# Fabstir/fabstir-vectordb

Hardware: AMD Instinct MI355X
Metric: k-NN queries/sec at recall@10>=0.95, 1Mx384 f32 (higher is better)
Workload: dtype f32

## Files before the change

fabstir-vectordb_amd/_capi.py:

```python
import ctypes as C
import os

_HERE = os.path.dirname(os.path.abspath(__file__))
LIB_DIR = os.environ.get("FVDB_LIB_DIR") or os.path.join(_HERE, "lib")
if not os.path.isabs(LIB_DIR):
    LIB_DIR = os.path.join(_HERE, LIB_DIR)
LIB_PATH = os.environ.get("FVDB_HIP_LIB") or os.path.join(LIB_DIR, "libfvdb_hip.so")

vp, u64, u32, i32, f32, sz = C.c_void_p, C.c_uint64, C.c_uint32, C.c_int, C.c_float, C.c_size_t
f32p, u64p, u32p = C.POINTER(C.c_float), C.POINTER(C.c_uint64), C.POINTER(C.c_uint32)


class TrainResult(C.Structure):
    _fields_ = [("iterations", u32), ("converged", u32), ("initial_error", f32), ("final_error", f32)]


class SearchStats(C.Structure):
    _fields_ = [("rows_scanned", u64), ("work_items", u64), ("list_rows_touched", u64)]


class MaskInfo(C.Structure):
    _fields_ = [("kind", u32), ("stale", u32), ("units", u32), ("reserved", u32), ("allowed_live", u64)]


# ... 23 lines not shown
    "fvdb_dev_upload": (i32, [vp, vp, vp, sz]),
    "fvdb_dev_download": (i32, [vp, vp, vp, sz]),
    "fvdb_timer_start": (i32, [vp]),
    "fvdb_timer_stop_ms": (i32, [vp, f32p]),
    "fvdb_ctx_set_profiling": (i32, [vp, i32]),
    "fvdb_dot_products": (i32, [vp, f32p, u32, f32p, u64, u32, f32p]),
    "fvdb_cosine_similarities": (i32, [vp, f32p, u32, f32p, u64, u32, f32p]),
    "fvdb_ivf_create": (i32, [vp, u32, u32, C.POINTER(vp)]),
    "fvdb_ivf_create_ex": (i32, [vp, u32, u32, i32, C.POINTER(vp)]),
    "fvdb_ivf_destroy": (None, [vp]),
    "fvdb_ivf_set_centroids": (i32, [vp, f32p]),
    "fvdb_ivf_get_centroids": (i32, [vp, f32p]),
    "fvdb_ivf_train": (i32, [vp, f32p, u64, u32, u64, C.POINTER(TrainResult)]),
    "fvdb_ivf_assign": (i32, [vp, f32p, u64, u32p]),
    "fvdb_ivf_add": (i32, [vp, f32p, u64p, u64, u32p, u32p]),
    "fvdb_ivf_add_assigned": (i32, [vp, f32p, u64p, u64, u32p, u32p]),
    "fvdb_ivf_set_deleted": (i32, [vp, u32p, u32p, u64, i32]),
    "fvdb_ivf_list_sizes": (i32, [vp, u64p]),
    "fvdb_ivf_list_export": (i32, [vp, u32, f32p, u64p, C.POINTER(C.c_uint8)]),
    "fvdb_ivf_total_rows": (u64, [vp]),
    "fvdb_ivf_reserve": (i32, [vp, u64]),
    "fvdb_ivf_clear": (i32, [vp]),
    "fvdb_ivf_set_global_list_sizes": (i32, [vp, u64p]),
    "fvdb_ivf_compact": (i32, [vp, u64p, u64p]),
    "fvdb_ivf_train_from": (i32, [vp, vp, u32, u64, C.POINTER(TrainResult)]),
    "fvdb_ivf_assign_from": (i32, [vp, vp, u32p, u64p]),
    "fvdb_ivf_refill_from": (i32, [vp, vp, u64, u32p]),
    "fvdb_ivf_maintenance_info": (i32, [vp, C.POINTER(MaintenanceInfo)]),
    "fvdb_ivf_get_rows": (i32, [vp, u32p, u32p, u64, f32p]),
    "fvdb_ivf_get_rows_dev": (i32, [vp, vp, u32p, u32p, u64, vp]),
    "fvdb_ivf_assign_from_store": (i32, [vp, vp, u32p, u64, u32p]),
    "fvdb_ivf_add_assigned_from_store": (i32, [vp, vp, u32p, u64p, u64, u32p, u32p]),
    "fvdb_ivf_search": (i32, [vp, f32p, u32, u32, u32, u64p, f32p, u32p]),
    "fvdb_ivf_search_dev": (i32, [vp, vp, u32, u32, u32, vp, vp, vp, vp]),
    "fvdb_ivf_search_all": (i32, [vp, f32p, u32, u32, u64p, f32p, u32p]),
    "fvdb_ivf_search_all_dev": (i32, [vp, vp, u32, u32, vp, vp, vp]),
    "fvdb_ivf_coarse": (i32, [vp, f32p, u32, u32, u32p, f32p]),
    "fvdb_ivf_set_coarse_mode": (i32, [vp, i32]),
    "fvdb_ivf_coarse_fallbacks": (i32, [vp, u64p]),
    "fvdb_ivf_set_scan_mode": (i32, [vp, i32]),
    "fvdb_ivf_scan_fallbacks": (i32, [vp, u64p]),
    "fvdb_ivf_scan_fallback_reasons": (i32, [vp, u64p]),
    "fvdb_ivf_scan_survivors": (i32, [vp, u32p, u32]),
    "fvdb_ivf_scan_survivor_dump": (i32, [vp, u32, u32, u32p, u32p, f32p, u32p]),
    "fvdb_ivf_last_stats": (i32, [vp, C.POINTER(SearchStats)]),
    "fvdb_ivf_stage_times": (u64, [vp, f32p]),
    "fvdb_ivf_profile_collect": (i32, [vp]),
    "fvdb_merge_keys_dev": (i32, [vp, vp, vp, u32, u32, u32, vp, vp, vp]),
    "fvdb_store_create": (i32, [vp, u32, u64, C.POINTER(vp)]),
    "fvdb_store_destroy": (None, [vp]),
    "fvdb_store_append": (i32, [vp, f32p, u64, u64p]),
    "fvdb_store_rows": (u64, [vp]),
    "fvdb_store_get": (i32, [vp, u64, f32p]),
    "fvdb_score_candidates": (i32, [vp, f32p, u32, u32p, u32, f32p]),
    "fvdb_scorer_create": (i32, [vp, u32, u32, C.POINTER(vp)]),
    "fvdb_scorer_destroy": (None, [vp]),
    "fvdb_scorer_set_queries": (i32, [vp, f32p, u32]),
    "fvdb_scorer_set_query_rows": (i32, [vp, u32p, u32]),
    "fvdb_scorer_set_queries_dev": (i32, [vp, vp, u32]),
    "fvdb_scorer_cand_buffer": (u32p, [vp]),
    "fvdb_scorer_dist_buffer": (f32p, [vp]),
    "fvdb_scorer_run": (i32, [vp, u32, u32]),
    "fvdb_graph_create": (i32, [vp, C.POINTER(vp)]),
    "fvdb_graph_destroy": (None, [vp]),
    "fvdb_graph_upload": (i32, [vp, u32, u32p, C.POINTER(C.c_uint8), u32p, u32p, u32]),
    "fvdb_graph_set_deleted": (i32, [vp, u32, i32]),
    "fvdb_graph_configure": (i32, [vp, u32, u32]),
    "fvdb_graph_append_nodes": (i32, [vp, u32, u32, u32p]),
    "fvdb_graph_insert_linked": (i32, [vp, u32, u32, u32, i32, u32p, vp]),
    "fvdb_graph_set_lists": (i32, [vp, u32, u32p, u32p, u32p, u32p]),
    "fvdb_graph_set_entry": (i32, [vp, u32, u32]),
    "fvdb_graph_entry": (i32, [vp, u32p, u32p]),
    "fvdb_graph_download": (i32, [vp, u32p, u32p, u64, u64p]),
    "fvdb_graph_upload_bytes": (u64, [vp]),
    "fvdb_graph_set_insert_visited": (i32, [vp, i32, u32]),
    "fvdb_graph_insert_info": (i32, [vp, u32, vp]),
    "fvdb_graph_vacuum": (i32, [vp, u32, u64p]),
    "fvdb_graph_maintenance_info": (i32, [vp, C.POINTER(GraphMaintenanceInfo)]),
    "fvdb_graph_search_dev": (i32, [vp, vp, u32, u32, u32, vp, vp, vp, vp]),
    "fvdb_graph_search_dev_slot": (i32, [vp, vp, u32, vp, u32, u32, u32, vp, vp, vp, vp]),
    "fvdb_ctx_device": (i32, [vp]),
    "fvdb_ctx_info": (i32, [vp, vp]),
    "fvdb_ivf_search_dev_slot": (i32, [vp, vp, u32, vp, u32, u32, u32, vp, vp, vp, vp]),
    "fvdb_ivf_coarse_dev_slot": (i32, [vp, vp, u32, vp, u32, u32, vp]),
    "fvdb_ivf_search_probes_dev_slot": (i32, [vp, vp, u32, vp, vp, u32, u32, u32, vp, vp, vp, vp]),
    "fvdb_host_alloc": (i32, [vp, C.c_size_t, C.POINTER(vp)]),
    "fvdb_host_free": (None, [vp, vp]),
    "fvdb_dev_download_async": (i32, [vp, vp, vp, C.c_size_t]),
    "fvdb_event_create": (i32, [vp, C.POINTER(vp)]),
    "fvdb_event_destroy": (None, [vp]),
    "fvdb_event_record": (i32, [vp, vp]),
    "fvdb_event_wait": (i32, [vp, vp]),
    "fvdb_graph_kernel_times": (i32, [vp, f32p, u32p, u64p, u64p]),
    "fvdb_graph_tie_restarts": (i32, [vp, u64p, u64p]),
    "fvdb_scorer_launch": (i32, [vp, u32, u32]),
    "fvdb_scorer_wait": (i32, [vp]),
    "fvdb_top_k_indices": (i32, [vp, f32p, u32, u64, u32, u64p, u32p]),
    "fvdb_top_k_indices_heap": (i32, [vp, f32p, u32, u64, u32, u64p, u32p]),
    "fvdb_top_k_indices_dev": (i32, [vp, vp, u32, u64, u32, i32, vp, vp]),
    "fvdb_streaming_top_k": (i32, [vp, u64p, f32p, u32, u64, u32, u64p, f32p, u32p]),
    "fvdb_streaming_top_k_dev": (i32, [vp, vp, vp, u32, u64, u32, vp, vp, vp]),
    "fvdb_merge_search_results": (i32, [vp, u64p, f32p, u32, u64, u32, u64p, f32p, u32p]),
    "fvdb_merge_search_results_dev": (i32, [vp, vp, vp, u32, u64, u32, vp, vp, vp]),
    "fvdb_comm_unique_id": (i32, [vp]),
    "fvdb_comm_create": (i32, [vp, vp, i32, i32, C.POINTER(vp)]),
    "fvdb_comm_create_hosted": (i32, [vp, i32, i32, vp, vp, C.POINTER(vp)]),
    "fvdb_comm_destroy": (None, [vp]),
    "fvdb_comm_rank": (i32, [vp]),
    "fvdb_comm_world": (i32, [vp]),
    "fvdb_comm_all_gather_dev": (i32, [vp, vp, vp, vp, sz]),
    "fvdb_comm_all_to_all_dev": (i32, [vp, vp, vp, vp, sz]),
    "fvdb_sharded_create": (i32, [vp, vp, C.POINTER(vp)]),
    "fvdb_sharded_destroy": (None, [vp]),
    "fvdb_sharded_out_rows": (u32, [vp, u32, i32]),
    "fvdb_ivf_search_sharded_begin": (i32, [vp, vp, u32, vp, u32, u32, u32, i32, vp, vp, vp]),
    "fvdb_ivf_search_sharded_end": (i32, [vp, vp, u32]),
    "fvdb_mask_create_ivf": (i32, [vp, u64p, u64, C.POINTER(vp)]),
    "fvdb_mask_create_graph": (i32, [vp, u32p, u64, C.POINTER(vp)]),
    "fvdb_mask_info": (i32, [vp, vp]),
    "fvdb_mask_destroy": (None, [vp]),
    "fvdb_ivf_search_dev_slot_masked": (i32, [vp, vp, u32, vp, vp, u32, u32, u32, vp, vp, vp, vp]),
    "fvdb_ivf_search_probes_dev_slot_masked": (i32, [vp, vp, u32, vp, vp, vp, u32, u32, u32, vp, vp, vp, vp]),
    "fvdb_ivf_search_wide_dev_slot": (i32, [vp, vp, u32, vp, vp, u32, u32, u32, vp, vp, vp, vp]),
    "fvdb_ivf_search_wide": (i32, [vp, f32p, u32, u32, u32, u64p, f32p, u32p]),
    "fvdb_ivf_search_quality_dev": (i32, [vp, vp, u32, vp, u32, u32, u32, vp, vp]),
    "fvdb_graph_search_dev_slot_masked": (i32, [vp, vp, u32, vp, vp, u32, u32, u32, vp, vp, vp, vp]),
    "fvdb_graph_scan_allowed_dev_slot": (i32, [vp, vp, u32, vp, vp, u32, u32, vp, vp, vp]),
}

_lib = None


def load():
    global _lib
    if _lib is not None:
        return _lib
    if not os.path.exists(LIB_PATH):
        raise ImportError(
            f"{LIB_PATH} not found: build it with `make -C fabstir-vectordb_amd` "
            "(or __graft_entry__.build()).  There is no CPU fallback.")
    os.environ.setdefault("GPU_MAX_HW_QUEUES", "16")
    lib = C.CDLL(LIB_PATH)
    for name, (res, args) in SIGNATURES.items():
        fn = getattr(lib, name)
        fn.restype = res
        fn.argtypes = args
    _lib = lib
    return lib
```

fabstir-vectordb_amd/csrc/fvdb_hip.cpp:

```cpp
#include "fvdb_internal.h"

#include <unistd.h>

#include <algorithm>
#include <atomic>
#include <cmath>
#include <condition_variable>
#include <mutex>
#include <cstdio>
#include <cstdlib>
#include <cstring>
#include <map>
#include <new>
#include <string>
#include <vector>

#include "common.h"
#include "kernels_misc.h"
#include "kernels_scan.h"
#include "kernels_wide.h"
#include "kernels_rank.h"
#include "kernels_coarse.h"
#include "kernels_mfma.h"
#include "kernels_mfma_wg.h"
// ... 40 lines not shown
    uint64_t* nv = nullptr;
    float* nn = nullptr;
    HIPCHK(ctx, hipMalloc(&nd, (size_t)ncap * block_bytes()));
    HIPCHK(ctx, hipMemsetAsync(nd, 0, (size_t)ncap * block_bytes(), ctx->stream));
    float* nr = nullptr;
    if (mirror && esize == 4) {
      HIPCHK(ctx, hipMalloc((void**)&nr, (size_t)ncap * block_bytes()));
      HIPCHK(ctx, hipMemsetAsync(nr, 0, (size_t)ncap * block_bytes(), ctx->stream));
      if (used_blocks && rm)
        HIPCHK(ctx, hipMemcpyAsync(nr, rm, (size_t)used_blocks * block_bytes(), hipMemcpyDeviceToDevice, ctx->stream));
    }
    void* nh = nullptr;
    if (mirror) {
      HIPCHK(ctx, hipMalloc(&nh, (size_t)ncap * block_bytes() / 2));
      HIPCHK(ctx, hipMemsetAsync(nh, 0, (size_t)ncap * block_bytes() / 2, ctx->stream));
      if (used_blocks && half)
        HIPCHK(ctx, hipMemcpyAsync(nh, half, (size_t)used_blocks * block_bytes() / 2, hipMemcpyDeviceToDevice, ctx->stream));
    }
    HIPCHK(ctx, hipMalloc(&nn, (size_t)ncap * 64 * sizeof(float)));
    HIPCHK(ctx, hipMemsetAsync(nn, 0, (size_t)ncap * 64 * sizeof(float), ctx->stream));
    HIPCHK(ctx, hipMalloc(&ni, (size_t)ncap * 64 * sizeof(uint64_t)));
    HIPCHK(ctx, hipMalloc(&nv, (size_t)ncap * sizeof(uint64_t)));
    HIPCHK(ctx, hipMemsetAsync(nv, 0, (size_t)ncap * sizeof(uint64_t), ctx->stream));
    if (used_blocks) {
      HIPCHK(ctx, hipMemcpyAsync(nd, data, (size_t)used_blocks * block_bytes(), hipMemcpyDeviceToDevice, ctx->stream));
      HIPCHK(ctx, hipMemcpyAsync(ni, ids, (size_t)used_blocks * 64 * sizeof(uint64_t), hipMemcpyDeviceToDevice,
                                 ctx->stream));
      HIPCHK(ctx, hipMemcpyAsync(nv, valid, (size_t)used_blocks * sizeof(uint64_t), hipMemcpyDeviceToDevice,
                                 ctx->stream));
      HIPCHK(ctx, hipMemcpyAsync(nn, norms, (size_t)used_blocks * 64 * sizeof(float), hipMemcpyDeviceToDevice,
                                 ctx->stream));
    }
    HIPCHK(ctx, hipStreamSynchronize(ctx->stream));
    if (data) (void)hipFree(data);
    if (ids) (void)hipFree(ids);
    if (valid) (void)hipFree(valid);
    if (norms) (void)hipFree(norms);
    if (half) (void)hipFree(half);
    half = nh;
    if (rm) (void)hipFree(rm);
    rm = nr;
    norms = nn;
    data = nd;
    ids = ni;
    valid = nv;
    cap_blocks = ncap;
    return FVDB_OK;
  }
};

enum FbWord : uint32_t {
  FB_COARSE = 0,
  FB_SCAN = 1,
  FB_REASONS = 2,
  FB_OVERFLOW = 2,
  FB_REFINED = 6,
  FB_WORDS = 8,
};
constexpr size_t kFbBytes = FB_WORDS * 4;
constexpr size_t kFbAllBytes = 2 * kFbBytes;
constexpr uint32_t kFbReasonWords = 5;

enum StageEvent {
  EV_COARSE_BEGIN = 0,
  EV_COARSE_SCANNED,
  EV_COARSE_DONE,
  EV_SCAN_BEGIN,
  EV_SCAN_DONE,
  EV_FINE_DONE,
  EV_FILTER_BEGIN,
  EV_FILTER_DONE,
  EV_COUNT
};

enum ScalWord : uint32_t {
  SC_COARSE_ITEMS = 0,
  SC_COARSE_HEAD = 1,
  SC_FINE_ITEMS = 2,
  SC_FINE_HEAD = 3,
  SC_STATS = 4,
};
constexpr size_t kScalarsBytes = 64;

struct IvfScratch {
  std::mutex enq;
  bool pend_filter = false;
  bool pending_profile = false, pend_coarse = false, pend_fine = false, collecting = false;
  std::vector<DBuf*> bufs;
  struct Buf : DBuf {
    explicit Buf(IvfScratch* set) { set->bufs.push_back(this); }
  };
  Buf s_qnorm{this}, s_A{this};
  Buf s_qh{this}, s_qn2{this}, s_thr{this}, s_tA{this}, s_pa{this}, s_surv{this}, s_scnt{this}, s_fail{this}, s_mslots{this};
  Buf s_sdist{this}, s_probes2{this};
  Buf s_q{this}, s_cpart{this}, s_probes{this}, s_cnt{this}, s_fill{this}, s_eoff{this}, s_ioff{this}, s_entries{this};
  Buf s_part{this}, s_scalars{this}, s_ceoff{this}, s_cioff{this};
  Buf s_wbase{this}, s_arena{this};
  Buf s_rbase{this}, s_rarena{this};
  Buf s_qual{this};
  Buf s_in{this}, s_slots{this}, s_ids{this}, s_clusters{this}, s_out_ids{this}, s_out_dist{this}, s_out_cnt{this}, s_cdist{this};
  Buf s_fslots{this}, s_frows{this};
  hipEvent_t fetch_done = nullptr;
  hipEvent_t sev[EV_COUNT] = {};
  uint32_t* scalar(ScalWord w) const { return s_scalars.as<uint32_t>() + w; }
  void release_all() {
    for (DBuf* b : bufs) b->release();
    if (fetch_done) (void)hipEventDestroy(fetch_done);
    fetch_done = nullptr;
    for (auto& e : sev) {
      if (e) (void)hipEventDestroy(e);
      e = nullptr;
    }
  }
};

struct fvdb_ivf : IvfScratch {
  static constexpr uint32_t kSlots = 16;
  IvfScratch spare[kSlots - 1];
  static constexpr uint32_t kLeases = 8;
  IvfScratch lease_set[kLeases];
  fvdb_ctx* lease_ctx[kLeases] = {};
  uint32_t lease_busy = 0;
  std::mutex mu;
  std::condition_variable lease_cv;
  std::atomic<IvfScratch*> last_set{nullptr};
  std::atomic<fvdb_ctx*> last_ctx{nullptr};
  fvdb_ctx* ctx = nullptr;
  uint32_t d = 0, dpad = 0, d4 = 0, nlist = 0;
  bool trained = false;
  bool f16 = false;

  std::vector<float> h_centroids;
  DBuf d_centroids_rm;
  DBuf d_cent_pad;
  DBuf d_cnorm, d_cnmax;
  DBuf s_fallbacks;
  uint32_t* fb_word(FbWord w, bool masked = false) const { return s_fallbacks.as<uint32_t>() + (masked ? FB_WORDS : 0) + w; }
  int coarse_mode = 0;
  int scan_mode = 0;
  HBuf h_fb;
  uint64_t mfma_q = 0;
  uint64_t fb_seen = 0, q_seen = 0;
  uint32_t exact_batches_left = 0;
  uint32_t backoff_len = 0;
  uint64_t overflow_seen = 0, overflow_q = 0;
  uint32_t refine_batches_left = 0;
  DBuf d_mfma_stamps;
  int mfma_stamps_launch = 0;
  DBuf d_xmax;
  Pool cpool;
  DBuf c_off, c_blocks, c_glob;

  Pool pool;
  std::vector<std::vector<uint32_t>> list_blocks;
  std::vector<uint32_t> list_len;
  uint64_t total_rows = 0;
  uint64_t mutations = 0;
  uint32_t max_list_blocks = 0;
  bool table_dirty = true;
  DBuf t_off, t_blocks, t_glob, t_len;
  std::vector<uint32_t> glob_blocks_host;
  bool glob_set = false;

  DBuf m_seq, m_dest, m_ids;
  fvdb_ivf* m_src = nullptr;
  uint64_t m_rows = 0;
  bool m_assigned = false;
  bool m_store_job = false;
  fvdb_maintenance_info_t m_info{};

  fvdb_search_stats last_stats{};
  float stage_ms[8] = {0, 0, 0, 0, 0, 0, 0, 0};
  uint64_t stage_calls = 0;
};

namespace {
struct Env {
  fvdb_ctx* ctx;
  IvfScratch* S;
  const uint64_t* live = nullptr;
};
inline IvfScratch& slot_scratch(fvdb_ivf* ivf, uint32_t slot) { return slot == 0 ? *ivf : ivf->spare[slot - 1]; }
inline const uint64_t* live_words(const fvdb_ivf* ivf, const Env& E) { return E.live ? E.live : ivf->pool.valid; }
inline PoolView list_pool(const fvdb_ivf* ivf, const Env& E) {
  PoolView v = ivf->pool.view();
  v.valid = live_words(ivf, E);
  return v;
}
}


namespace {

struct IvfKnobs {
  static int num(const char* name, int unset) { return getenv(name) ? atoi(getenv(name)) : unset; }
  static bool has(const char* name) { return getenv(name) != nullptr; }
  static int tiles(int m) { return m >= 4 ? 4 : (m >= 2 ? 2 : 1); }
  bool coarse_exact = has("FVDB_COARSE_EXACT");
  bool scan_exact = has("FVDB_SCAN_EXACT");
  uint32_t scan_wgs_per_cu = (uint32_t)num("FVDB_SCAN_WGS_PER_CU", 8);
  int segb = num("FVDB_SEGB", 0);
  bool no_shared_thr = has("FVDB_NO_SHARED_THR");
  int mfma_m = tiles(num("FVDB_MFMA_M", 2));
  int mfma_segb = num("FVDB_MFMA_SEGB", 0);
  uint32_t mfma_wgs_per_cu = (uint32_t)std::max(1, num("FVDB_MFMA_WGS_PER_CU", 2));
  bool mfma_groups_in_item = num("FVDB_MFMA_GROUPS_IN_ITEM", 0) != 0;
  bool mfma_wg = num("FVDB_MFMA_WG", 1) != 0;
  int mfma_wg_m = num("FVDB_MFMA_WG_M", 4) >= 4 ? 4 : 2;
  uint32_t mfma_wg_segb = (uint32_t)std::max(4, num("FVDB_MFMA_WG_SEGB", 16));
  uint32_t mfma_wg_per_cu = (uint32_t)std::max(1, num("FVDB_MFMA_WG_PER_CU", 2));
  int mfma_wg_tail_pct = num("FVDB_MFMA_WG_TAIL_PCT", 25);
  int mfma_wg_segb_tail = num("FVDB_MFMA_WG_SEGB_TAIL", 4);
  uint32_t mfma_cap_a = (uint32_t)std::max(1, num("FVDB_MFMA_CAP_A", 4));
  bool mfma_threshold_pass = has("FVDB_MFMA_THRESHOLD_PASS");
  uint32_t mfma_segb_a = (uint32_t)std::max(1, num("FVDB_MFMA_SEGB_A", 1));
  bool mfma_no_refine = has("FVDB_MFMA_NO_REFINE");
#ifdef FVDB_MFMA_STAMPS_BUILD
  int mfma_stamps = num("FVDB_MFMA_STAMPS", 0);
#endif
};
const IvfKnobs& ivf_knobs() {
  static const IvfKnobs knobs{};
  return knobs;
}

struct ScanLaunch {
  PoolView pool;
  const uint32_t* list_off;
  const uint32_t* list_blocks;
  uint32_t nlist;
  const uint32_t* entry_off;
  const uint32_t* item_off;
  const uint2* entries;
  const uint32_t* n_items;
  uint32_t* head;
  const float* queries;
  uint32_t dpad, segb, k, nprobe, maxsegs;
  uint2* part;
  uint32_t max_items = 0;
  bool f16 = false;
};

inline int kr_for(uint32_t k) { return k <= 64 ? 1 : (k <= 128 ? 2 : 4); }
inline uint32_t q_for(uint32_t k) { return k <= 64 ? 16u : (k <= 128 ? 8u : 4u); }

template <int Q, int KR, int ROLE, int ST>
void launch_scan_t(fvdb_ctx* ctx, const ScanLaunch& s) {
  uint32_t grid = (uint32_t)ctx->num_cus * ivf_knobs().scan_wgs_per_cu;
  if (s.max_items) grid = std::min(grid, std::max<uint32_t>(1u, (s.max_items + 3) / 4));
  hipLaunchKernelGGL((scan_topk_kernel<Q, KR, ROLE, ST>), dim3(grid), dim3(256), 0, ctx->stream, s.pool.data, s.pool.valid,
                     s.pool.d4, s.list_off, s.list_blocks, s.nlist, s.entry_off, s.item_off, (const u32x2*)s.entries,
                     s.n_items, s.head, s.queries, s.dpad, s.segb, s.k, s.nprobe, s.maxsegs, (u32x2*)s.part);
}

template <int ROLE, int ST>
void launch_scan_rs(fvdb_ctx* ctx, const ScanLaunch& s) {
  switch (kr_for(s.k)) {
    case 1: launch_scan_t<16, 1, ROLE, ST>(ctx, s); break;
    case 2: launch_scan_t<8, 2, ROLE, ST>(ctx, s); break;
    default: launch_scan_t<4, 4, ROLE, ST>(ctx, s); break;
  }
}
template <int ROLE>
void launch_scan_r(fvdb_ctx* ctx, const ScanLaunch& s) {
  if (s.f16) launch_scan_rs<ROLE, 1>(ctx, s); else launch_scan_rs<ROLE, 0>(ctx, s);
}
enum { ROLE_COARSE = 0, ROLE_LIST = 1, ROLE_ALL = 2 };
void launch_scan(fvdb_ctx* ctx, const ScanLaunch& s, int role) {
  if (role == ROLE_COARSE) launch_scan_r<ROLE_COARSE>(ctx, s);
  else if (role == ROLE_LIST) launch_scan_r<ROLE_LIST>(ctx, s);
  else launch_scan_r<ROLE_ALL>(ctx, s);
}

void launch_merge(fvdb_ctx* ctx, const MergeArgs& m) {
  const uint32_t grid = cdiv(m.B, 4);
  switch (kr_for(m.k)) {
    case 1: hipLaunchKernelGGL((merge_topk_kernel<1>), dim3(grid), dim3(256), 0, ctx->stream, m); break;
    case 2: hipLaunchKernelGGL((merge_topk_kernel<2>), dim3(grid), dim3(256), 0, ctx->stream, m); break;
    default: hipLaunchKernelGGL((merge_topk_kernel<4>), dim3(grid), dim3(256), 0, ctx->stream, m); break;
  }
}

int upload_table(fvdb_ivf* ivf) {
  fvdb_ctx* ctx = ivf->ctx;
  std::lock_guard<std::mutex> lk(ivf->mu);
  if (!ivf->table_dirty) return FVDB_OK;
  std::vector<uint32_t> off(ivf->nlist + 1, 0), blocks;
  std::vector<uint32_t> glob(ivf->nlist, 0);
  uint32_t mx = 0;
  for (uint32_t L = 0; L < ivf->nlist; ++L) {
    off[L] = (uint32_t)blocks.size();
    blocks.insert(blocks.end(), ivf->list_blocks[L].begin(), ivf->list_blocks[L].end());
    mx = std::max<uint32_t>(mx, (uint32_t)ivf->list_blocks[L].size());
    glob[L] = ivf->glob_set ? ivf->glob_blocks_host[L] : (uint32_t)ivf->list_blocks[L].size();
  }
  off[ivf->nlist] = (uint32_t)blocks.size();
  ivf->max_list_blocks = mx;
  HIPCHK(ctx, ivf->t_off.ensure(off.size() * 4));
  HIPCHK(ctx, ivf->t_blocks.ensure(std::max<size_t>(blocks.size(), 1) * 4));
  HIPCHK(ctx, ivf->t_glob.ensure(glob.size() * 4));
  HIPCHK(ctx, hipMemcpyAsync(ivf->t_off.p, off.data(), off.size() * 4, hipMemcpyHostToDevice, ctx->stream));
  if (!blocks.empty())
    HIPCHK(ctx, hipMemcpyAsync(ivf->t_blocks.p, blocks.data(), blocks.size() * 4, hipMemcpyHostToDevice, ctx->stream));
  HIPCHK(ctx, hipMemcpyAsync(ivf->t_glob.p, glob.data(), glob.size() * 4, hipMemcpyHostToDevice, ctx->stream));
  HIPCHK(ctx, ivf->t_len.ensure((size_t)ivf->nlist * 4));
  HIPCHK(ctx, hipMemcpyAsync(ivf->t_len.p, ivf->list_len.data(), (size_t)ivf->nlist * 4, hipMemcpyHostToDevice,
                             ctx->stream));
  HIPCHK(ctx, hipStreamSynchronize(ctx->stream));
  ivf->table_dirty = false;
  return FVDB_OK;
}

int padded_queries(fvdb_ivf* ivf, const Env& E, const float* q_dev, uint32_t B, const float** out) {
  fvdb_ctx* ctx = E.ctx;
  IvfScratch& S = *E.S;
  if (ivf->d == ivf->dpad) {
    *out = q_dev;
    return FVDB_OK;
  }
  HIPCHK(ctx, S.s_q.ensure((size_t)B * ivf->dpad * 4));
  const uint64_t tot = (uint64_t)B * ivf->dpad;
  hipLaunchKernelGGL(pad_rows_kernel, dim3(cdiv(tot, 256)), dim3(256), 0, ctx->stream, q_dev, ivf->d, ivf->dpad,
                     (uint64_t)B, S.s_q.as<float>());
  *out = S.s_q.as<float>();
  return FVDB_OK;
}

inline void mark(const fvdb_ivf* ivf, const Env& E, StageEvent e) {
  if (ivf->ctx->profiling) (void)hipEventRecord(E.S->sev[e], E.ctx->stream);
}

struct Batch {
  const float* qpad;
  const uint32_t* probes;
  uint32_t B, k, np;
  uint64_t* out_ids;
  float* out_dist;
  uint32_t* out_counts;
  uint64_t* out_keys;
  const float* given_thr = nullptr;
};

inline ListTable list_table(const fvdb_ivf* ivf) {
  return ListTable{ivf->t_off.as<uint32_t>(), ivf->t_blocks.as<uint32_t>(), ivf->nlist};
}

MergeArgs merge_args(const PoolView& pool, const ListTable& lists, const uint32_t* glob_blocks, const DBuf& part,
                     uint32_t maxsegs, uint32_t segb, const Batch& b) {
  MergeArgs m{};
  m.pool = pool;
  m.lists = lists;
  m.probes = b.probes;
  m.glob_blocks = glob_blocks;
  m.part = part.as<uint2>();
  m.B = b.B;
  m.k = b.k;
  m.nprobe = b.np;
  m.maxsegs = maxsegs;
  m.segb = segb;
  m.out_ids = b.out_ids;
  m.out_dist = b.out_dist;
  m.out_counts = b.out_counts;
  m.out_keys = b.out_keys;
  return m;
}

constexpr uint64_t kRankArenaBytes = 256ull << 20;
int check_rank(fvdb_ctx* ctx, const fvdb_ivf* ivf, uint32_t np) {
  if (np > FVDB_MAX_K && ivf->nlist > kRankSortMaxLists)
    FAIL(ctx, FVDB_E_UNSUPPORTED, "nprobe above FVDB_MAX_K needs an index of at most 16384 lists");
  return FVDB_OK;
}

int run_coarse_rank(fvdb_ivf* ivf, const Env& E, const float* qpad, uint32_t B, uint32_t kc, uint32_t* out_probes,
                    float* out_dist) {
  fvdb_ctx* ctx = E.ctx;
  IvfScratch& S = *E.S;
  int rc = check_rank(ctx, ivf, kc);
  if (rc) return rc;
  const uint32_t cblocks = ivf->cpool.used_blocks, n = cblocks * 64;
  uint32_t P = 1;
  while (P < n) P <<= 1;
  const uint32_t lds = P * 8;
  const uint32_t threads = std::min<uint32_t>(kRankThreads, std::max<uint32_t>(64, P / 2));
  const uint32_t chunk = (uint32_t)std::min<uint64_t>(B, std::max<uint64_t>(1, kRankArenaBytes / ((uint64_t)n * 4)));
  HIPCHK(ctx, S.s_rarena.ensure((size_t)chunk * n * 4));
  HIPCHK(ctx, S.s_rbase.ensure((size_t)chunk * 2 * 4));
  HIPCHK(ctx, S.s_entries.ensure((size_t)chunk * 8));
  HIPCHK(ctx, S.s_ceoff.ensure(16));
  HIPCHK(ctx, S.s_cioff.ensure(16));
  HIPCHK(ctx, S.s_scalars.ensure(kScalarsBytes));
  HIPCHK(ctx, hipFuncSetAttribute((const void*)rank_sort_kernel, hipFuncAttributeMaxDynamicSharedMemorySize,
                                  (int)(kRankSortMaxLists * 8)));
  const ListTable clist{ivf->c_off.as<uint32_t>(), ivf->c_blocks.as<uint32_t>(), 1};
  const PoolView cpool = ivf->cpool.view();
  const uint32_t grid = (uint32_t)ctx->num_cus * ivf_knobs().scan_wgs_per_cu;
  mark(ivf, E, EV_COARSE_BEGIN);
  for (uint32_t o = 0; o < B; o += chunk) {
    const uint32_t b = std::min(chunk, B - o);
    hipLaunchKernelGGL(plan_all_kernel, dim3(cdiv(b, 256)), dim3(256), 0, ctx->stream, b, cblocks, 1u, 16u,
                       S.s_ceoff.as<uint32_t>(), S.s_cioff.as<uint32_t>(), S.s_entries.as<uint2>(),
                       S.scalar(SC_COARSE_ITEMS), S.scalar(SC_COARSE_HEAD));
    hipLaunchKernelGGL(rank_base_kernel, dim3(cdiv(b, 256)), dim3(256), 0, ctx->stream, b, cblocks, S.s_rbase.as<uint32_t>());
    const uint32_t items = cblocks * cdiv(b, 16);
    hipLaunchKernelGGL(wide_score_kernel<0>, dim3(std::min(grid, std::max<uint32_t>(1u, cdiv(items, 4)))), dim3(256), 0,
                       ctx->stream, cpool.data, cpool.valid, cpool.d4, clist.off, clist.blocks, 1u, S.s_ceoff.as<uint32_t>(),
                       S.s_cioff.as<uint32_t>(), (const u32x2*)S.s_entries.as<uint2>(), S.scalar(SC_COARSE_ITEMS),
                       S.scalar(SC_COARSE_HEAD), qpad + (size_t)o * ivf->dpad, ivf->dpad, 1u, 1u, S.s_rbase.as<uint32_t>(),
                       S.s_rarena.as<uint32_t>(), (uint64_t)n);
    if (o + b == B) mark(ivf, E, EV_COARSE_SCANNED);
    RankArgs r{};
    r.pool = cpool;
    r.lists = clist;
    r.arena = S.s_rarena.as<uint32_t>();
    r.n = n;
    r.P = P;
    r.np = kc;
    r.out_probes = out_probes + (size_t)o * kc;
    r.out_dist = out_dist ? out_dist + (size_t)o * kc : nullptr;
    hipLaunchKernelGGL(rank_sort_kernel, dim3(b), dim3(threads), lds, ctx->stream, r);
  }
  mark(ivf, E, EV_COARSE_DONE);
  HIPCHK(ctx, hipGetLastError());
  return FVDB_OK;
// ... 7 lines not shown
  if (ivf->coarse_mode == 0 && !ivf_knobs().coarse_exact && ivf->dpad % 16 == 0 && kc <= 48 && ivf->nlist >= 64 && B > 0 &&
      (uint64_t)B * ivf->nlist < (1ull << 31)) {
    const uint32_t nlist = ivf->nlist;
    const float* cpad = ivf->d == ivf->dpad ? ivf->d_centroids_rm.as<float>() : ivf->d_cent_pad.as<float>();
    HIPCHK(ctx, S.s_qnorm.ensure((size_t)B * 4));
    HIPCHK(ctx, S.s_A.ensure((size_t)B * nlist * 4));
    mark(ivf, E, EV_COARSE_BEGIN);
    hipLaunchKernelGGL(row_sqnorm_wave_kernel, dim3(cdiv(B, 4)), dim3(256), 0, ctx->stream, qpad, ivf->dpad, ivf->dpad, B,
                       S.s_qnorm.as<float>());
    const uint32_t waves = cdiv(B, 32) * cdiv(nlist, 64);
    hipLaunchKernelGGL(coarse_gemm_kernel, dim3(cdiv(waves, 4)), dim3(256), 0, ctx->stream, qpad, cpad,
                       S.s_qnorm.as<float>(), ivf->d_cnorm.as<float>(), B, nlist, ivf->dpad, S.s_A.as<float>());
    mark(ivf, E, EV_COARSE_SCANNED);
    hipLaunchKernelGGL(coarse_select_kernel, dim3(cdiv(B, 4)), dim3(256), 0, ctx->stream, S.s_A.as<float>(), qpad, cpad,
                       S.s_qnorm.as<float>(), ivf->d_cnmax.as<float>(), B, nlist, ivf->d, ivf->dpad, 64u, kc,
                       out_probes, out_dist, ivf->fb_word(FB_COARSE));
    mark(ivf, E, EV_COARSE_DONE);
    HIPCHK(ctx, hipGetLastError());
    return FVDB_OK;
  }
  const uint32_t cblocks = ivf->cpool.used_blocks;
  const uint32_t segb = 1, Q = q_for(kc);
  const uint32_t maxsegs = cblocks;
  HIPCHK(ctx, S.s_cpart.ensure((size_t)B * maxsegs * kc * 8));
  HIPCHK(ctx, S.s_entries.ensure((size_t)B * std::max<uint32_t>(kc, 1) * 8));
  HIPCHK(ctx, S.s_ceoff.ensure(16));
  HIPCHK(ctx, S.s_cioff.ensure(16));
  HIPCHK(ctx, S.s_scalars.ensure(kScalarsBytes));
  hipLaunchKernelGGL(plan_all_kernel, dim3(cdiv(std::max<uint32_t>(B, 1), 256)), dim3(256), 0, ctx->stream, B, cblocks,
                     segb, Q, S.s_ceoff.as<uint32_t>(), S.s_cioff.as<uint32_t>(), S.s_entries.as<uint2>(),
                     S.scalar(SC_COARSE_ITEMS), S.scalar(SC_COARSE_HEAD));
  const ListTable clist{ivf->c_off.as<uint32_t>(), ivf->c_blocks.as<uint32_t>(), 1};
  ScanLaunch s{ivf->cpool.view(), clist.off, clist.blocks, 1, S.s_ceoff.as<uint32_t>(), S.s_cioff.as<uint32_t>(),
               S.s_entries.as<uint2>(), S.scalar(SC_COARSE_ITEMS), S.scalar(SC_COARSE_HEAD), qpad, ivf->dpad, segb, kc, 1,
               maxsegs, S.s_cpart.as<uint2>(), cdiv(cblocks, segb) * cdiv(B, Q)};
  mark(ivf, E, EV_COARSE_BEGIN);
  launch_scan(ctx, s, ROLE_COARSE);
  mark(ivf, E, EV_COARSE_SCANNED);
  MergeArgs m = merge_args(ivf->cpool.view(), clist, ivf->c_glob.as<uint32_t>(), S.s_cpart, maxsegs, segb,
                           Batch{qpad, nullptr, B, kc, 1, nullptr, out_dist, nullptr, nullptr});
  m.out_probes = out_probes;
  launch_merge(ctx, m);
  mark(ivf, E, EV_COARSE_DONE);
  HIPCHK(ctx, hipGetLastError());
  return FVDB_OK;
}

uint32_t segb_for(uint32_t max_blocks, uint32_t B, uint32_t nprobe) {
  const uint64_t pairs = (uint64_t)B * nprobe;
  if (max_blocks >= 4096) return 16;
  if (pairs >= 4096) return 4;
  if (pairs >= 512) return 2;
  return 1;
}
uint32_t pick_segb(fvdb_ivf* ivf, uint32_t B, uint32_t nprobe) {
  const int forced = ivf_knobs().segb;
  return forced > 0 ? (uint32_t)forced : segb_for(ivf->max_list_blocks, B, nprobe);
}
uint64_t queries_per_gib(uint32_t max_blocks, uint32_t segb, uint32_t k, uint32_t np) {
  const uint64_t per_q = (uint64_t)np * std::max<uint32_t>(1, cdiv(max_blocks, segb)) * k * 8;
  return (1ull << 30) / std::max<uint64_t>(per_q, 1);
}

void launch_plan(fvdb_ivf* ivf, const Env& E, const uint32_t* probes, uint32_t n, uint32_t np, uint32_t segb, uint32_t Q,
                 unsigned long long* stats, uint32_t* rezero_cnt, uint32_t lsplit = 0xFFFFFFFFu, uint32_t segb_tail = 0) {
  fvdb_ctx* ctx = E.ctx;
  IvfScratch& S = *E.S;
  const uint32_t* list_off = ivf->t_off.as<uint32_t>();
  hipLaunchKernelGGL(plan_count_kernel, dim3(cdiv(n, 256)), dim3(256), 0, ctx->stream, probes, n, S.s_cnt.as<uint32_t>(),
                     list_off);
  hipLaunchKernelGGL(plan_scan_kernel, dim3(1), dim3(1024), 0, ctx->stream, S.s_cnt.as<uint32_t>(), list_off,
                     ivf->t_len.as<uint32_t>(), ivf->nlist, segb, Q, S.s_eoff.as<uint32_t>(), S.s_ioff.as<uint32_t>(),
                     S.s_fill.as<uint32_t>(), S.scalar(SC_FINE_ITEMS), S.scalar(SC_FINE_HEAD), stats, rezero_cnt, lsplit,
                     segb_tail);
  hipLaunchKernelGGL(plan_fill_kernel, dim3(cdiv(n, 256)), dim3(256), 0, ctx->stream, probes, n, np,
                     S.s_eoff.as<uint32_t>(), S.s_fill.as<uint32_t>(), S.s_entries.as<uint2>(), list_off);
}
inline unsigned long long* scan_stats(const IvfScratch& S) { return (unsigned long long*)S.scalar(SC_STATS); }

int plan_scratch(fvdb_ivf* ivf, const Env& E, uint32_t B, uint32_t np) {
  fvdb_ctx* ctx = E.ctx;
  IvfScratch& S = *E.S;
  const uint32_t nlist = ivf->nlist;
  HIPCHK(ctx, S.s_cnt.ensure((size_t)nlist * 4));
  HIPCHK(ctx, S.s_fill.ensure((size_t)nlist * 4));
  HIPCHK(ctx, S.s_eoff.ensure((size_t)(nlist + 1) * 4));
  HIPCHK(ctx, S.s_ioff.ensure((size_t)(nlist + 1) * 4));
  HIPCHK(ctx, S.s_entries.ensure((size_t)B * np * 8));
  return FVDB_OK;
}

int run_fine_exact(fvdb_ivf* ivf, const Env& E, const Batch& b, int role) {
  fvdb_ctx* ctx = E.ctx;
  IvfScratch& S = *E.S;
  const uint32_t nlist = ivf->nlist;
  const uint32_t segb = pick_segb(ivf, b.B, b.np), Q = q_for(b.k);
  const uint32_t maxsegs = std::max<uint32_t>(1, cdiv(ivf->max_list_blocks, segb));
  const uint64_t part_elems = (uint64_t)b.B * b.np * maxsegs * b.k;
  if (part_elems >= (1ull << 32)) FAIL(ctx, FVDB_E_UNSUPPORTED, "batch too large for one launch (sub-batch it)");
  int rc = plan_scratch(ivf, E, b.B, b.np);
  if (rc) return rc;
  HIPCHK(ctx, S.s_part.ensure((size_t)part_elems * 8));
  HIPCHK(ctx, S.s_scalars.ensure(kScalarsBytes));
  HIPCHK(ctx, hipMemsetAsync(S.s_cnt.p, 0, (size_t)nlist * 4, ctx->stream));
  launch_plan(ivf, E, b.probes, b.B * b.np, b.np, segb, Q, scan_stats(S), nullptr);
  mark(ivf, E, EV_SCAN_BEGIN);
  const ListTable lists = list_table(ivf);
  ScanLaunch s{list_pool(ivf, E), lists.off, lists.blocks, nlist, S.s_eoff.as<uint32_t>(), S.s_ioff.as<uint32_t>(),
               S.s_entries.as<uint2>(), S.scalar(SC_FINE_ITEMS), S.scalar(SC_FINE_HEAD), b.qpad, ivf->dpad, segb, b.k, b.np,
               maxsegs, S.s_part.as<uint2>()};
  s.f16 = ivf->f16;
  launch_scan(ctx, s, role);
  mark(ivf, E, EV_SCAN_DONE);
  launch_merge(ctx, merge_args(list_pool(ivf, E), lists, ivf->t_glob.as<uint32_t>(), S.s_part, maxsegs, segb, b));
  mark(ivf, E, EV_FINE_DONE);
  HIPCHK(ctx, hipGetLastError());
  return FVDB_OK;
}

constexpr uint32_t kMfmaSlack = 6;
constexpr uint32_t kMfmaCmax = 4096;

bool mfma_shape_ok(const fvdb_ivf* ivf, uint32_t B, uint32_t k, uint32_t np) {
  return ivf->dpad % 16 == 0 && k + kMfmaSlack <= 32 && np <= 256 && B >= 32 && B <= 16384;
}
inline bool half_rows(const fvdb_ivf* ivf) { return ivf->f16 || ivf->pool.half != nullptr; }
inline int x_rounded(const fvdb_ivf* ivf) { return ivf->f16 ? 0 : (ivf->pool.half ? 1 : 2); }

struct MfmaPlan {
  bool wg;
  int M;
  uint32_t Q, ka, cmax;
  uint32_t segb, segbA;
  uint32_t lsplit, segb_tail;
  uint32_t fsegb, fmaxsegs;
  uint64_t fpart;
  uint32_t grid, wg_grid, wg_lds;
  bool half_rows;
  int x_rounded;
};

int mfma_plan(fvdb_ivf* ivf, fvdb_ctx* ctx, const IvfKnobs& kn, uint32_t B, uint32_t k, uint32_t np, MfmaPlan* out) {
  MfmaPlan P{};
  P.half_rows = half_rows(ivf);
  P.x_rounded = x_rounded(ivf);
  int wgM = kn.mfma_wg_m;
  if (mfma_wg_lds_bytes(ivf->dpad, 16u * wgM) > 64u * 1024u) wgM = 2;
  P.wg = kn.mfma_wg && kn.mfma_m == 2 && P.half_rows && ivf->dpad % 128 == 0 &&
         mfma_wg_lds_bytes(ivf->dpad, 16u * wgM) <= 64u * 1024u;
  P.M = P.wg ? wgM : kn.mfma_m;
  P.Q = 16u * P.M;
  P.ka = k + kMfmaSlack;
  P.cmax = kMfmaCmax;
  P.segbA = kn.mfma_segb_a;
  P.segb = P.wg ? kn.mfma_wg_segb : (kn.mfma_segb > 0 ? (uint32_t)kn.mfma_segb : pick_segb(ivf, B, np));
  P.lsplit = 0xFFFFFFFFu;
  P.segb_tail = P.segb;
  if (P.wg && kn.mfma_wg_tail_pct > 0 && kn.mfma_wg_segb_tail > 0 && (uint32_t)kn.mfma_wg_segb_tail < P.segb) {
    P.lsplit = (uint32_t)((uint64_t)ivf->nlist * (uint32_t)(100 - std::min(kn.mfma_wg_tail_pct, 100)) / 100);
    P.segb_tail = (uint32_t)kn.mfma_wg_segb_tail;
  }
  P.fsegb = pick_segb(ivf, B, np);
  P.fmaxsegs = std::max<uint32_t>(1, cdiv(ivf->max_list_blocks, P.fsegb));
  P.fpart = (uint64_t)B * np * P.fmaxsegs * k;
  if (P.fpart >= (1ull << 32)) FAIL(ctx, FVDB_E_UNSUPPORTED, "batch too large for one launch (sub-batch it)");
  P.grid = (uint32_t)ctx->num_cus * kn.mfma_wgs_per_cu;
  P.wg_grid = (uint32_t)ctx->num_cus * kn.mfma_wg_per_cu;
  P.wg_lds = mfma_wg_lds_bytes(ivf->dpad, P.Q);
  *out = P;
  return FVDB_OK;
}

int mfma_scratch(fvdb_ivf* ivf, const Env& E, const MfmaPlan& P, uint32_t B, uint32_t np) {
  fvdb_ctx* ctx = E.ctx;
  IvfScratch& S = *E.S;
  HIPCHK(ctx, S.s_qh.ensure((size_t)(B + 1) * ivf->dpad * 2));
  HIPCHK(ctx, S.s_qn2.ensure((size_t)B * 4));
  HIPCHK(ctx, S.s_thr.ensure((size_t)B * 4));
  HIPCHK(ctx, S.s_tA.ensure((size_t)B * 4));
  HIPCHK(ctx, S.s_pa.ensure((size_t)B * 4));
  HIPCHK(ctx, S.s_mslots.ensure((size_t)B * 64 * 4));
  HIPCHK(ctx, S.s_surv.ensure((size_t)B * P.cmax * 8));
  HIPCHK(ctx, S.s_sdist.ensure((size_t)B * P.cmax * 4));
  HIPCHK(ctx, S.s_scnt.ensure((size_t)(B + 2) * 4));
  HIPCHK(ctx, S.s_fail.ensure((size_t)B * 4));
  HIPCHK(ctx, S.s_part.ensure((size_t)P.fpart * 8));
  int rc = plan_scratch(ivf, E, B, np);
  if (rc) return rc;
  HIPCHK(ctx, S.s_scalars.ensure(kScalarsBytes));
  return FVDB_OK;
}

void launch_prep_queries(fvdb_ivf* ivf, const Env& E, const float* qpad, uint32_t B) {
  IvfScratch& S = *E.S;
  hipLaunchKernelGGL(prep_queries_kernel, dim3(cdiv(B + 1, 4)), dim3(256), 0, E.ctx->stream, qpad, B, ivf->dpad,
                     (_Float16*)S.s_qh.p, S.s_qn2.as<float>(), S.s_cnt.as<uint32_t>(), ivf->nlist,
                     S.s_scnt.as<uint32_t>(), S.s_mslots.as<uint32_t>());
}

ThresholdArgs threshold_args(fvdb_ivf* ivf, const Env& E, const float* qpad, const uint32_t* probes, uint32_t B,
                             uint32_t k, uint32_t np, float* thr_out) {
  const IvfScratch& S = *E.S;
  ThresholdArgs t{};
  t.rows = ivf->pool.half ? ivf->pool.half : ivf->pool.data;
  t.pool_valid = live_words(ivf, E);
  t.pool_norms = ivf->pool.norms;
  t.d4 = ivf->d4;
  t.lists = list_table(ivf);
  t.list_len = ivf->t_len.as<uint32_t>();
  t.probes = probes;
  t.qh = (const _Float16*)S.s_qh.p;
  t.queries = qpad;
  t.qn = S.s_qn2.as<float>();
  t.xmax_bits = ivf->d_xmax.as<uint32_t>();
  t.B = B;
  t.np = np;
  t.ka = k + kMfmaSlack;
  t.dpad = ivf->dpad;
  t.capA = ivf_knobs().mfma_cap_a;
  t.min_rows = 256u;
  t.rows_f16 = x_rounded(ivf);
  t.thr = thr_out;
  return t;
}
void launch_threshold_direct(fvdb_ivf* ivf, fvdb_ctx* ctx, const ThresholdArgs& t) {
  if (half_rows(ivf)) hipLaunchKernelGGL((threshold_direct_kernel<true>), dim3(cdiv(t.B, 4)), dim3(256), 0, ctx->stream, t);
  else hipLaunchKernelGGL((threshold_direct_kernel<false>), dim3(cdiv(t.B, 4)), dim3(256), 0, ctx->stream, t);
}

MfmaScanArgs mfma_scan_args(fvdb_ivf* ivf, const Env& E, const MfmaPlan& P, const Batch& b) {
  const IvfScratch& S = *E.S;
  MfmaScanArgs a{};
  a.pool_data = ivf->pool.half ? ivf->pool.half : ivf->pool.data;
  a.pool_valid = live_words(ivf, E);
  a.pool_norms = ivf->pool.norms;
  a.d4 = ivf->d4;
  a.list_off = ivf->t_off.as<uint32_t>();
  a.list_blocks = ivf->t_blocks.as<uint32_t>();
  a.nlist = ivf->nlist;
  a.entry_off = S.s_eoff.as<uint32_t>();
  a.item_off = S.s_ioff.as<uint32_t>();
  a.entries = (const u32x2*)S.s_entries.p;
  a.n_items = S.scalar(SC_FINE_ITEMS);
  a.head = S.scalar(SC_FINE_HEAD);
  a.qh = (const _Float16*)S.s_qh.p;
  a.zero_row = b.B;
  a.dpad = ivf->dpad;
  a.segb = P.segb;
  a.thr = b.given_thr ? b.given_thr : S.s_thr.as<float>();
  a.cmax = P.cmax;
  a.surv = (u32x2*)S.s_surv.p;
  a.sval = S.s_sdist.as<float>();
  a.scnt = S.s_scnt.as<uint32_t>();
  a.slots = S.s_mslots.as<uint32_t>();
  a.capA = ivf_knobs().mfma_cap_a;
  a.groups_in_item = ivf_knobs().mfma_groups_in_item ? 1u : 0u;
  a.lsplit = P.lsplit;
  a.segb_tail = P.segb_tail;
  return a;
}

using MfmaKernel = decltype(&scan_mfma_kernel<2, 1, 0>);
template <int M, int MODE>
MfmaKernel mfma_kernel_of(bool f16) {
  return f16 ? scan_mfma_kernel<M, 1, MODE> : scan_mfma_kernel<M, 0, MODE>;
}
template <int MODE>
void launch_mfma(fvdb_ctx* ctx, const MfmaScanArgs& a, const MfmaPlan& P) {
  const MfmaKernel kernel = P.M == 1   ? mfma_kernel_of<1, MODE>(P.half_rows)
                            : P.M == 2 ? mfma_kernel_of<2, MODE>(P.half_rows)
                                       : mfma_kernel_of<4, MODE>(P.half_rows);
  hipLaunchKernelGGL(kernel, dim3(P.grid), dim3(256), 0, ctx->stream, a);
}

void mfma_threshold(fvdb_ivf* ivf, const Env& E, const MfmaPlan& P, const Batch& b, const MfmaScanArgs& a) {
  fvdb_ctx* ctx = E.ctx;
  IvfScratch& S = *E.S;
  if (b.given_thr) return;
  if (!ivf_knobs().mfma_threshold_pass) {
    launch_threshold_direct(ivf, ctx, threshold_args(ivf, E, b.qpad, b.probes, b.B, b.k, b.np, S.s_thr.as<float>()));
    return;
  }
  hipLaunchKernelGGL(first_probe_kernel, dim3(cdiv(b.B, 256)), dim3(256), 0, ctx->stream, b.probes, b.B, b.np,
                     ivf->t_len.as<uint32_t>(), 256u, S.s_pa.as<uint32_t>());
  launch_plan(ivf, E, S.s_pa.as<uint32_t>(), b.B, 1, P.segbA, P.Q, nullptr, S.s_cnt.as<uint32_t>());
  MfmaScanArgs head = a;
  head.segb = P.segbA;
  launch_mfma<1>(ctx, head, P);
  hipLaunchKernelGGL(threshold_kernel, dim3(cdiv(b.B, 4)), dim3(256), 0, ctx->stream, S.s_mslots.as<uint32_t>(),
                     S.s_pa.as<uint32_t>(), S.s_qn2.as<float>(), ivf->d_xmax.as<uint32_t>(), b.B, P.ka, ivf->dpad,
                     P.x_rounded, S.s_thr.as<float>());
}

void launch_filter(fvdb_ctx* ctx, const MfmaScanArgs& a, const MfmaPlan& P) {
  if (P.wg) {
    const MfmaKernel kernel = P.M == 4 ? scan_mfma_wg_kernel<4> : scan_mfma_wg_kernel<2>;
    hipLaunchKernelGGL(kernel, dim3(P.wg_grid), dim3(256), P.wg_lds, ctx->stream, a);
  } else {
    launch_mfma<0>(ctx, a, P);
  }
}

#ifdef FVDB_MFMA_STAMPS_BUILD
constexpr uint32_t kStampsCap = 32768;
int mfma_stamps_begin(fvdb_ivf* ivf, fvdb_ctx* ctx, const MfmaPlan& P, MfmaScanArgs* a) {
  const int stamps_env = ivf_knobs().mfma_stamps;
  const bool stamp_now = P.wg && stamps_env && ++ivf->mfma_stamps_launch >= stamps_env && ivf->mfma_stamps_launch < stamps_env + 3;
  if (!stamp_now) return FVDB_OK;
  HIPCHK(ctx, ivf->d_mfma_stamps.ensure((size_t)kStampsCap * 64));
  HIPCHK(ctx, hipMemsetAsync(ivf->d_mfma_stamps.p, 0, (size_t)kStampsCap * 64, ctx->stream));
  a->stamps = ivf->d_mfma_stamps.as<unsigned long long>();
  a->stamps_cap = kStampsCap;
  return FVDB_OK;
}
int mfma_stamps_report(fvdb_ivf* ivf, fvdb_ctx* ctx, MfmaScanArgs* a) {
  if (!a->stamps) return FVDB_OK;
  HIPCHK(ctx, hipStreamSynchronize(ctx->stream));
  std::vector<unsigned long long> h((size_t)kStampsCap * 8);
  HIPCHK(ctx, hipMemcpy(h.data(), a->stamps, h.size() * 8, hipMemcpyDeviceToHost));
  unsigned long long t_min = ~0ull, t_max = 0;
  size_t n = 0;
  for (size_t i = 0; i < kStampsCap; ++i)
    if (h[i * 8 + 3]) {
      t_min = std::min(t_min, h[i * 8]);
      t_max = std::max(t_max, h[i * 8 + 3]);
      ++n;
    }
  double s_loc = 0, s_tile = 0, s_comp = 0, s_steps = 0, s_blocks = 0;
  size_t per_xcd[16] = {0};
  std::vector<double> per_step;
  for (size_t i = 0; i < kStampsCap; ++i) {
    const unsigned long long* r = &h[i * 8];
    if (!r[3]) continue;
    const double steps = (double)((r[5] + 3) / 4) * (double)(ivf->dpad / 16);
    s_loc += (double)(r[1] - r[0]);
    s_tile += (double)(r[2] - r[1]);
    s_comp += (double)(r[3] - r[2]);
    s_steps += steps;
    s_blocks += (double)r[5];
    per_xcd[r[7] & 15]++;
    per_step.push_back((double)(r[3] - r[2]) / steps);
  }
  std::sort(per_step.begin(), per_step.end());
  const double tick = 0.01;
  fprintf(stderr,
          "[mfma stamps] launch %d: %zu items, %0.f blocks, span %.1f us | per item (wave 0): locate %.2f us, tile %.2f us, "
          "compute %.2f us | per 16-dim step: mean %.3f us, p10 %.3f, p50 %.3f, p90 %.3f | items per XCD",
          ivf->mfma_stamps_launch, n, s_blocks, (double)(t_max - t_min) * tick, s_loc / n * tick, s_tile / n * tick, s_comp / n * tick,
          s_comp / s_steps * tick, per_step.empty() ? 0.0 : per_step[per_step.size() / 10] * tick,
          per_step.empty() ? 0.0 : per_step[per_step.size() / 2] * tick,
          per_step.empty() ? 0.0 : per_step[per_step.size() * 9 / 10] * tick);
  for (int x = 0; x < 8; ++x) fprintf(stderr, " %zu", per_xcd[x]);
  unsigned long long last_start = 0;
  for (size_t i = 0; i < kStampsCap; ++i)
    if (h[i * 8 + 3]) last_start = std::max(last_start, h[i * 8]);
  fprintf(stderr, " | last item drawn at %.1f us\n", (double)(last_start - t_min) * tick);
  a->stamps = nullptr;
  return FVDB_OK;
}
#else
inline int mfma_stamps_begin(fvdb_ivf*, fvdb_ctx*, const MfmaPlan&, MfmaScanArgs*) { return FVDB_OK; }
inline int mfma_stamps_report(fvdb_ivf*, fvdb_ctx*, MfmaScanArgs*) { return FVDB_OK; }
#endif

int mfma_filter(fvdb_ivf* ivf, const Env& E, const MfmaPlan& P, const Batch& b, MfmaScanArgs* a) {
  fvdb_ctx* ctx = E.ctx;
  launch_plan(ivf, E, b.probes, b.B * b.np, b.np, P.segb, P.Q, scan_stats(*E.S), E.S->s_cnt.as<uint32_t>(), P.lsplit,
              P.segb_tail);
  mark(ivf, E, EV_FILTER_BEGIN);
  int rc = mfma_stamps_begin(ivf, ctx, P, a);
  if (rc) return rc;
  launch_filter(ctx, *a, P);
  rc = mfma_stamps_report(ivf, ctx, a);
  if (rc) return rc;
  mark(ivf, E, EV_FILTER_DONE);
  return FVDB_OK;
}

bool auto_backs_off(fvdb_ivf* ivf) {
  std::lock_guard<std::mutex> lk(ivf->mu);
  if (ivf->exact_batches_left > 0) {
    ivf->exact_batches_left -= 1;
    return true;
  }
  if (!(ivf->h_fb.p && ivf->mfma_q - ivf->q_seen >= 2048)) return false;
  const uint64_t fb_now = ((volatile uint32_t*)ivf->h_fb.p)[FB_SCAN];
  const uint64_t dq = ivf->mfma_q - ivf->q_seen, dfb = fb_now - ivf->fb_seen;
  ivf->q_seen = ivf->mfma_q;
  ivf->fb_seen = fb_now;
  if (dfb * 8 > dq) {
    ivf->backoff_len = std::min<uint32_t>(ivf->backoff_len ? ivf->backoff_len * 2 : 64, 4096);
    ivf->exact_batches_left = ivf->backoff_len;
    return true;
  }
  ivf->backoff_len = 0;
  return false;
}
bool auto_refines(fvdb_ivf* ivf) {
  std::lock_guard<std::mutex> lk(ivf->mu);
  if (ivf->h_fb.p && ivf->mfma_q - ivf->overflow_q >= 2048) {
    const volatile uint32_t* c = (const volatile uint32_t*)ivf->h_fb.p;
    const uint64_t now = (uint64_t)c[FB_OVERFLOW] + c[FB_REFINED], dq = ivf->mfma_q - ivf->overflow_q;
    if ((now - ivf->overflow_seen) * 1000 > dq) ivf->refine_batches_left = 1024;
    ivf->overflow_seen = now;
    ivf->overflow_q = ivf->mfma_q;
  }
  if (ivf->refine_batches_left == 0) return false;
  ivf->refine_batches_left -= 1;
  return true;
}

int mfma_refine(fvdb_ivf* ivf, const Env& E, const MfmaPlan& P, const Batch& b, const MfmaScanArgs& a) {
  fvdb_ctx* ctx = E.ctx;
  IvfScratch& S = *E.S;
  HIPCHK(ctx, S.s_probes2.ensure((size_t)b.B * b.np * 4));
  hipLaunchKernelGGL(refine_threshold_kernel, dim3(cdiv(b.B, 4)), dim3(256), 0, ctx->stream, S.s_sdist.as<float>(),
                     S.s_scnt.as<uint32_t>(), b.probes, S.s_qn2.as<float>(), ivf->d_xmax.as<uint32_t>(), b.B, b.np, P.ka, P.cmax,
                     ivf->dpad, P.x_rounded, S.s_thr.as<float>(), S.s_probes2.as<uint32_t>(), ivf->fb_word(FB_REFINED, E.live != nullptr));
  launch_plan(ivf, E, S.s_probes2.as<uint32_t>(), b.B * b.np, b.np, P.segb, P.Q, nullptr, S.s_cnt.as<uint32_t>(), P.lsplit,
              P.segb_tail);
  launch_filter(ctx, a, P);
  return FVDB_OK;
}

VerifyArgs verify_args(fvdb_ivf* ivf, const Env& E, const MfmaPlan& P, const Batch& b) {
  const IvfScratch& S = *E.S;
  VerifyArgs v{};
  v.pool = list_pool(ivf, E);
  v.lists = list_table(ivf);
  v.probes = b.probes;
  v.glob_blocks = ivf->t_glob.as<uint32_t>();
  v.queries = b.qpad;
  v.qn = S.s_qn2.as<float>();
  v.xmax_bits = ivf->d_xmax.as<uint32_t>();
  v.thr = b.given_thr ? b.given_thr : S.s_thr.as<float>();
  v.remote_thr = b.given_thr ? 1 : 0;
  v.surv = (const u32x2*)S.s_surv.p;
  v.sval = S.s_sdist.as<float>();
  v.scnt = S.s_scnt.as<uint32_t>();
  v.B = b.B;
  v.k = b.k;
  v.ka = P.ka;
  v.nprobe = b.np;
  v.d = ivf->dpad;
  v.dpad = ivf->dpad;
  v.cmax = P.cmax;
  v.rows_f16 = P.x_rounded;
  v.rows_rm = ivf->pool.rm;
  v.out_ids = b.out_ids;
  v.out_dist = b.out_dist;
  v.out_counts = b.out_counts;
  v.out_keys = b.out_keys;
  v.fallbacks = ivf->fb_word(FB_SCAN, E.live != nullptr);
  v.reasons = ivf->fb_word(FB_REASONS, E.live != nullptr);
  v.fail_list = S.s_fail.as<uint32_t>();
  v.nfail = S.s_scnt.as<uint32_t>() + b.B;
  return v;
}
void launch_select(fvdb_ivf* ivf, fvdb_ctx* ctx, const VerifyArgs& v) {
  if (ivf->f16) hipLaunchKernelGGL((select_kernel<1>), dim3(cdiv(v.B, 4)), dim3(256), 0, ctx->stream, v);
  else hipLaunchKernelGGL((select_kernel<0>), dim3(cdiv(v.B, 4)), dim3(256), 0, ctx->stream, v);
}

FallbackArgs fallback_args(fvdb_ivf* ivf, const Env& E, const MfmaPlan& P, const Batch& b, const VerifyArgs& v) {
  const IvfScratch& S = *E.S;
  FallbackArgs fa{};
  fa.pool = list_pool(ivf, E);
  fa.lists = v.lists;
  fa.probes = b.probes;
  fa.queries = b.qpad;
  fa.fail_list = v.fail_list;
  fa.nfail = v.nfail;
  fa.head = S.s_scnt.as<uint32_t>() + b.B + 1;
  fa.k = b.k;
  fa.nprobe = b.np;
  fa.dpad = ivf->dpad;
  fa.segb = P.fsegb;
  fa.maxsegs = P.fmaxsegs;
  fa.part = (u32x2*)S.s_part.p;
  return fa;
}

void mfma_rescan(fvdb_ivf* ivf, const Env& E, const MfmaPlan& P, const Batch& b, const VerifyArgs& v) {
  fvdb_ctx* ctx = E.ctx;
  const FallbackArgs fa = fallback_args(ivf, E, P, b, v);
  if (ivf->f16) hipLaunchKernelGGL((fallback_scan_kernel<1>), dim3(P.grid), dim3(256), 0, ctx->stream, fa);
  else hipLaunchKernelGGL((fallback_scan_kernel<0>), dim3(P.grid), dim3(256), 0, ctx->stream, fa);
  MergeArgs fm = merge_args(fa.pool, fa.lists, v.glob_blocks, E.S->s_part, P.fmaxsegs, P.fsegb, b);
  fm.qlist = v.fail_list;
  fm.nq = v.nfail;
  launch_merge(ctx, fm);
}

int mfma_watch_counters(fvdb_ivf* ivf, fvdb_ctx* ctx, uint32_t B) {
  {
    std::lock_guard<std::mutex> lk(ivf->mu);
    const bool fresh = ivf->h_fb.p == nullptr;
    HIPCHK(ctx, ivf->h_fb.ensure(64));
    if (fresh) std::memset(ivf->h_fb.p, 0, 64);
    ivf->mfma_q += B;
  }
  HIPCHK(ctx, hipMemcpyAsync(ivf->h_fb.p, ivf->s_fallbacks.p, kFbBytes, hipMemcpyDeviceToHost, ctx->stream));
  return FVDB_OK;
}

int run_fine_mfma(fvdb_ivf* ivf, const Env& E, const Batch& b) {
  fvdb_ctx* ctx = E.ctx;
  const IvfKnobs& kn = ivf_knobs();
  MfmaPlan P;
  int rc = mfma_plan(ivf, ctx, kn, b.B, b.k, b.np, &P);
  if (rc) return rc;
  rc = mfma_scratch(ivf, E, P, b.B, b.np);
  if (rc) return rc;
  mark(ivf, E, EV_SCAN_BEGIN);
  launch_prep_queries(ivf, E, b.qpad, b.B);
  MfmaScanArgs a = mfma_scan_args(ivf, E, P, b);
  mfma_threshold(ivf, E, P, b, a);
  rc = mfma_filter(ivf, E, P, b, &a);
  if (rc) return rc;
  if (!b.given_thr && !kn.mfma_no_refine && (ivf->scan_mode != FVDB_SCAN_AUTO || auto_refines(ivf))) {
    rc = mfma_refine(ivf, E, P, b, a);
    if (rc) return rc;
  }
  mark(ivf, E, EV_SCAN_DONE);
  E.S->pend_filter = true;
  const VerifyArgs v = verify_args(ivf, E, P, b);
  launch_select(ivf, ctx, v);
  mfma_rescan(ivf, E, P, b, v);
  mark(ivf, E, EV_FINE_DONE);
  if (!E.live) {
    rc = mfma_watch_counters(ivf, ctx, b.B);
    if (rc) return rc;
  }
  HIPCHK(ctx, hipGetLastError());
  return FVDB_OK;
}

int run_fine(fvdb_ivf* ivf, const Env& E, const Batch& b, int role) {
  E.S->pend_filter = false;
  bool mfma = (ivf->scan_mode == FVDB_SCAN_AUTO || ivf->scan_mode == FVDB_SCAN_FILTER) && !ivf_knobs().scan_exact &&
              mfma_shape_ok(ivf, b.B, b.k, b.np) && role == ROLE_LIST && ivf->pool.norms != nullptr;
  if (mfma && E.live && ivf->scan_mode == FVDB_SCAN_AUTO) mfma = false;
  if (mfma && ivf->scan_mode == FVDB_SCAN_AUTO && auto_backs_off(ivf)) mfma = false;
  if (mfma) return run_fine_mfma(ivf, E, b);
  return run_fine_exact(ivf, E, b, role);
}

struct StageSpan {
  StageEvent from, to;
};
constexpr StageSpan kStageSpan[6] = {
    {EV_COARSE_BEGIN, EV_COARSE_SCANNED}, {EV_COARSE_SCANNED, EV_COARSE_DONE},
    {EV_COARSE_DONE, EV_SCAN_BEGIN},
    {EV_SCAN_BEGIN, EV_SCAN_DONE},        {EV_SCAN_DONE, EV_FINE_DONE},
    {EV_FILTER_BEGIN, EV_FILTER_DONE}};

int finish_profile(fvdb_ivf* ivf, const Env& E, bool coarse, bool fine) {
  fvdb_ctx* ctx = E.ctx;
  IvfScratch& S = *E.S;
  if (!ivf->ctx->profiling) return FVDB_OK;
  if (ivf->ctx->profiling == 2 && !S.collecting) {
    S.pend_coarse = coarse;
    S.pend_fine = fine;
    S.pending_profile = true;
    return FVDB_OK;
  }
  HIPCHK(ctx, hipStreamSynchronize(ctx->stream));
  float ms = 0;
  auto add = [&](int stage) {
    (void)hipEventElapsedTime(&ms, S.sev[kStageSpan[stage].from], S.sev[kStageSpan[stage].to]);
    ivf->stage_ms[stage] += ms;
  };
  if (coarse) {
    add(0);
    add(1);
  }
  if (fine) {
    if (coarse) add(2);
    add(3);
    add(4);
    if (S.pend_filter) add(5);
  }
  ivf->stage_calls += 1;
  return FVDB_OK;
}

uint32_t sub_batch(fvdb_ivf* ivf, uint32_t B, uint32_t k, uint32_t np) {
  uint64_t fit = queries_per_gib(ivf->max_list_blocks, pick_segb(ivf, B, np), k, np);
  fit = std::max<uint64_t>(fit, 1);
  fit = std::min<uint64_t>(fit, 16384);
  return (uint32_t)std::min<uint64_t>(fit, B);
}

static_assert(kWideMaxK == FVDB_MAX_K_WIDE && kWideMaxProbes == FVDB_MAX_K, "kernels_wide.h sizes its LDS by these");
constexpr uint64_t kWideArenaBytes = 1ull << 30;
uint32_t wide_arena_blocks(const fvdb_ivf* ivf, uint32_t np) {
  const uint64_t all = ivf->pool.used_blocks;
  return (uint32_t)std::max<uint64_t>(1, std::min<uint64_t>((uint64_t)np * ivf->max_list_blocks, all));
}
uint32_t wide_sub_batch(const fvdb_ivf* ivf, uint32_t B, uint32_t np) {
  const uint64_t per_q = (uint64_t)wide_arena_blocks(ivf, np) * 256;
  const uint64_t fit = std::min<uint64_t>(std::max<uint64_t>(kWideArenaBytes / per_q, 1), 16384);
  return (uint32_t)std::min<uint64_t>(fit, B);
}

int run_fine_wide(fvdb_ivf* ivf, const Env& E, const Batch& b) {
  fvdb_ctx* ctx = E.ctx;
  IvfScratch& S = *E.S;
  S.pend_filter = false;
  const uint32_t nlist = ivf->nlist;
  const uint32_t segb = pick_segb(ivf, b.B, b.np);
  const uint32_t cap_blocks = wide_arena_blocks(ivf, b.np);
  const uint64_t stride = (uint64_t)cap_blocks * 64;
  int rc = plan_scratch(ivf, E, b.B, b.np);
  if (rc) return rc;
  HIPCHK(ctx, S.s_wbase.ensure((size_t)b.B * (b.np + 1) * 4));
  HIPCHK(ctx, S.s_arena.ensure((size_t)b.B * stride * 4));
  HIPCHK(ctx, S.s_scalars.ensure(kScalarsBytes));
  HIPCHK(ctx, hipMemsetAsync(S.s_cnt.p, 0, (size_t)nlist * 4, ctx->stream));
  launch_plan(ivf, E, b.probes, b.B * b.np, b.np, segb, 16, scan_stats(S), nullptr);
  const ListTable lists = list_table(ivf);
  hipLaunchKernelGGL(wide_base_kernel, dim3(cdiv(b.B, 256)), dim3(256), 0, ctx->stream, b.probes, lists.off, b.B, b.np,
                     cap_blocks, S.s_wbase.as<uint32_t>());
  mark(ivf, E, EV_SCAN_BEGIN);
  const PoolView pool = list_pool(ivf, E);
  const uint32_t grid = (uint32_t)ctx->num_cus * ivf_knobs().scan_wgs_per_cu;
  auto score = ivf->f16 ? wide_score_kernel<1> : wide_score_kernel<0>;
  hipLaunchKernelGGL(score, dim3(grid), dim3(256), 0, ctx->stream, pool.data, pool.valid, pool.d4, lists.off, lists.blocks,
                     nlist, S.s_eoff.as<uint32_t>(), S.s_ioff.as<uint32_t>(), (const u32x2*)S.s_entries.as<uint2>(),
                     S.scalar(SC_FINE_ITEMS), S.scalar(SC_FINE_HEAD), b.qpad, ivf->dpad, segb, b.np,
                     S.s_wbase.as<uint32_t>(), S.s_arena.as<uint32_t>(), stride);
  mark(ivf, E, EV_SCAN_DONE);
  WideArgs w{};
  w.pool = pool;
  w.lists = lists;
  w.probes = b.probes;
  w.base = S.s_wbase.as<uint32_t>();
  w.arena = S.s_arena.as<uint32_t>();
  w.stride = stride;
  w.B = b.B;
  w.k = b.k;
  w.nprobe = b.np;
  w.out_ids = b.out_ids;
  w.out_dist = b.out_dist;
  w.out_counts = b.out_counts;
  w.out_keys = b.out_keys;
  if (b.np <= kWideMaxProbes)
    hipLaunchKernelGGL(wide_select_kernel<true>, dim3(b.B), dim3(kWideSelThreads), 0, ctx->stream, w);
  else
    hipLaunchKernelGGL(wide_select_kernel<false>, dim3(b.B), dim3(kWideSelThreads), 0, ctx->stream, w);
  mark(ivf, E, EV_FINE_DONE);
  HIPCHK(ctx, hipGetLastError());
  return FVDB_OK;
}

bool thr_share_ok(fvdb_ivf* ivf, uint32_t B, uint32_t k, uint32_t np) {
  const IvfKnobs& kn = ivf_knobs();
  if (kn.scan_exact || kn.no_shared_thr || ivf->scan_mode != FVDB_SCAN_AUTO) return false;
  if (!mfma_shape_ok(ivf, B, k, np)) return false;
  uint32_t gmax = 0;
  if (ivf->glob_set) {
    for (uint32_t b : ivf->glob_blocks_host) gmax = std::max(gmax, b);
  } else {
    gmax = ivf->max_list_blocks;
  }
  return queries_per_gib(gmax, segb_for(gmax, B, np), k, np) >= B;
}

int ivf_shared_thresholds(fvdb_ivf* ivf, const Env& E, const float* q_dev, const uint32_t* probes, uint32_t B, uint32_t k,
                          uint32_t np, float* u_out) {
  fvdb_ctx* ctx = E.ctx;
  IvfScratch& S = *E.S;
  HIPCHK(ctx, hipSetDevice(ctx->device));
  int rc = upload_table(ivf);
  if (rc) return rc;
  std::lock_guard<std::mutex> enq(S.enq);
  HIPCHK(ctx, S.s_qn2.ensure((size_t)B * 4));
  if (!ivf->pool.norms || !ivf->d_xmax.p) {
    HIPCHK(ctx, hipMemsetAsync(S.s_qn2.p, 0, (size_t)B * 4, ctx->stream));
    hipLaunchKernelGGL(fill_f32_kernel, dim3(cdiv(B, 256)), dim3(256), 0, ctx->stream, u_out, (uint64_t)B, __builtin_huge_valf());
    HIPCHK(ctx, hipGetLastError());
    return FVDB_OK;
  }
  const float* qpad = nullptr;
  rc = padded_queries(ivf, E, q_dev, B, &qpad);
  if (rc) return rc;
  HIPCHK(ctx, S.s_qh.ensure((size_t)(B + 1) * ivf->dpad * 2));
  HIPCHK(ctx, S.s_cnt.ensure((size_t)ivf->nlist * 4));
  HIPCHK(ctx, S.s_scnt.ensure((size_t)(B + 2) * 4));
  HIPCHK(ctx, S.s_mslots.ensure((size_t)B * 64 * 4));
  launch_prep_queries(ivf, E, qpad, B);
  ThresholdArgs t = threshold_args(ivf, E, qpad, probes, B, k, np, u_out);
  t.glob_blocks = ivf->t_glob.as<uint32_t>();
  launch_threshold_direct(ivf, ctx, t);
  HIPCHK(ctx, hipGetLastError());
  return FVDB_OK;
}

int ivf_thr_combine(fvdb_ivf* ivf, const Env& E, const float* u_all, uint32_t W, uint32_t B, float* thr_out,
                    bool loopback_fill = false) {
  fvdb_ctx* ctx = E.ctx;
  IvfScratch& S = *E.S;
  if (!ivf->d_xmax.p) {
    HIPCHK(ctx, ivf->d_xmax.ensure(4));
    HIPCHK(ctx, hipMemsetAsync(ivf->d_xmax.p, 0, 4, ctx->stream));
  }
  hipLaunchKernelGGL(thr_combine_kernel, dim3(cdiv(B, 256)), dim3(256), 0, ctx->stream, u_all, W, B, S.s_qn2.as<float>(),
                     ivf->d_xmax.as<uint32_t>(), (float)ivf->dpad, x_rounded(ivf), thr_out);
#ifdef FVDB_DEV_TOOLS
  if (loopback_fill)
    hipLaunchKernelGGL(thr_loopback_fill_kernel, dim3(1), dim3(1024), 0, ctx->stream, thr_out, S.s_qn2.as<float>(), B);
#else
  (void)loopback_fill;
#endif
  HIPCHK(ctx, hipGetLastError());
  return FVDB_OK;
}

int check_finite(fvdb_ctx* ctx, const float* x, uint64_t n) {
  for (uint64_t i = 0; i < n; ++i)
    if (!std::isfinite(x[i])) FAIL(ctx, FVDB_E_NONFINITE, "non-finite input value");
  return FVDB_OK;
}

}

static std::mutex g_hwq_mu;
static int g_hwq_state = 0, g_hwq_value = 0;
static bool hip_runtime_already_up() {
  char path[64], tgt[256];
  for (int fd = 0; fd < 1024; ++fd) {
    snprintf(path, sizeof path, "/proc/self/fd/%d", fd);
    const ssize_t n = readlink(path, tgt, sizeof tgt - 1);
    if (n <= 0) continue;
    tgt[n] = 0;
    if (strstr(tgt, "/dev/kfd")) return true;
  }
  return false;
}

extern "C" {

const char* fvdb_version(void) { return "fvdb-hip 0.1 (gfx950)"; }

int fvdb_ctx_create(int device, fvdb_ctx** out) {
  if (!out) return FVDB_E_INVALID;
  *out = nullptr;
  {
    std::lock_guard<std::mutex> lk(g_hwq_mu);
    if (g_hwq_state == 0) {
      const char* set = getenv("GPU_MAX_HW_QUEUES");
      if (set) {
        g_hwq_value = atoi(set);
        g_hwq_state = 1;
      } else if (hip_runtime_already_up()) {
        g_hwq_value = 4;
        g_hwq_state = 3;
        fprintf(stderr, "[fvdb] warning: HIP was initialised before fvdb_ctx_create, so GPU_MAX_HW_QUEUES=16 cannot be applied; "
                        "with the default of 4 hardware queues batches in flight overlap less (export GPU_MAX_HW_QUEUES=16 before "
                        "the process touches the GPU)\n");
      } else {
        (void)setenv("GPU_MAX_HW_QUEUES", "16", 0);
        g_hwq_value = 16;
        g_hwq_state = 2;
      }
    }
  }
  int ndev = 0;
  if (hipGetDeviceCount(&ndev) != hipSuccess || ndev <= 0 || device < 0 || device >= ndev) return FVDB_E_HIP;
  fvdb_ctx* ctx = new (std::nothrow) fvdb_ctx();
  if (!ctx) return FVDB_E_OOM;
// ... 480 lines not shown
  std::vector<uint32_t> cl(n);
  HIPCHK(ctx, hipMemcpyAsync(cl.data(), ivf->s_clusters.p, n * 4, hipMemcpyDeviceToHost, ctx->stream));
  HIPCHK(ctx, hipStreamSynchronize(ctx->stream));
  if (out_cluster) std::memcpy(out_cluster, cl.data(), n * 4);
  return append_staged(ivf, ids, n, cl.data(), out_pos);
}

int fvdb_ivf_set_deleted(fvdb_ivf* ivf, const uint32_t* cluster, const uint32_t* pos, uint64_t n, int deleted) {
  fvdb_ctx* ctx = ivf->ctx;
  if (n == 0) return FVDB_OK;
  ivf->mutations += 1;
  HIPCHK(ctx, hipSetDevice(ctx->device));
  std::vector<uint32_t> slots(n);
  for (uint64_t i = 0; i < n; ++i) {
    if (cluster[i] >= ivf->nlist || pos[i] >= ivf->list_len[cluster[i]]) FAIL(ctx, FVDB_E_NOT_FOUND, "no such row");
    slots[i] = ivf->list_blocks[cluster[i]][pos[i] >> 6] * 64 + (pos[i] & 63);
  }
  HIPCHK(ctx, ivf->s_slots.ensure(n * 4));
  HIPCHK(ctx, hipMemcpyAsync(ivf->s_slots.p, slots.data(), n * 4, hipMemcpyHostToDevice, ctx->stream));
  hipLaunchKernelGGL(set_valid_kernel, dim3(cdiv(n, 256)), dim3(256), 0, ctx->stream, ivf->s_slots.as<uint32_t>(), n,
                     deleted, (unsigned long long*)ivf->pool.valid);
  HIPCHK(ctx, hipGetLastError());
  HIPCHK(ctx, hipStreamSynchronize(ctx->stream));
  return FVDB_OK;
}

extern "C++" {
namespace {
struct IvfSearch {
  enum Kind {
    PROBED,
    ALL,
    WIDE,
    COARSE_ONLY,
  } kind;
  const float* q_dev;
  uint32_t B, k, nprobe;
  uint64_t* ids = nullptr;
  float* dist = nullptr;
  uint32_t* counts = nullptr;
  uint64_t* keys = nullptr;
  const uint32_t* given_probes = nullptr;
  const float* given_thr = nullptr;
  uint32_t* probes_out = nullptr;

  IvfSearch slice(uint32_t o, uint32_t b, uint32_t d, uint32_t np) const {
    auto at = [o](auto* p, size_t stride) { return p ? p + (size_t)o * stride : nullptr; };
    IvfSearch s = *this;
    s.B = b;
    s.q_dev = at(q_dev, d);
    s.ids = at(ids, k);
    s.dist = at(dist, k);
    s.counts = at(counts, 1);
    s.keys = at(keys, k);
    s.given_probes = at(given_probes, np);
    s.given_thr = at(given_thr, 1);
    s.probes_out = at(probes_out, np);
    return s;
  }
};

inline bool wide_route(IvfSearch::Kind kind, uint32_t np) {
  return kind == IvfSearch::WIDE || (kind == IvfSearch::PROBED && np > FVDB_MAX_K);
}
inline uint32_t probed_lists(const fvdb_ivf* ivf, IvfSearch::Kind kind, uint32_t nprobe) {
  return kind == IvfSearch::ALL ? ivf->nlist : std::min(nprobe, ivf->nlist);
}

int check_k(fvdb_ctx* ctx, IvfSearch::Kind kind, uint32_t k, uint32_t np) {
  if (wide_route(kind, np)) {
    if (k == 0 || k > FVDB_MAX_K_WIDE) FAIL(ctx, FVDB_E_UNSUPPORTED, "k must be in 1..FVDB_MAX_K_WIDE");
  } else if (k == 0 || k > FVDB_MAX_K) {
    FAIL(ctx, FVDB_E_UNSUPPORTED, "k must be in 1..FVDB_MAX_K");
  }
  return FVDB_OK;
}

void ensure_stage_events(const fvdb_ivf* ivf, IvfScratch& S) {
  if (!ivf->ctx->profiling) return;
  for (auto& e : S.sev)
    if (!e) (void)hipEventCreate(&e);
}

int ivf_search(fvdb_ivf* ivf, const Env& E, const IvfSearch& R) {
  fvdb_ctx* ctx = E.ctx;
  IvfScratch& S = *E.S;
  const uint32_t np = probed_lists(ivf, R.kind, R.nprobe);
  const bool all = R.kind == IvfSearch::ALL, wide = wide_route(R.kind, np);
  if (!ivf->trained) FAIL(ctx, FVDB_E_NOT_TRAINED, "index not trained");
  int rc = check_k(ctx, R.kind, R.k, np);
  if (rc) return rc;
  if (wide && ivf->glob_set)
    FAIL(ctx, FVDB_E_UNSUPPORTED, "the wide search (k or nprobe above FVDB_MAX_K) does not serve a shard of a larger index");
  if (R.B == 0) return FVDB_OK;
  HIPCHK(ctx, hipSetDevice(ctx->device));
  if (np == 0) FAIL(ctx, FVDB_E_INVALID, "nprobe must be > 0");
  if (!all && (rc = check_rank(ctx, ivf, np))) return rc;
  rc = upload_table(ivf);
  if (rc) return rc;
  std::lock_guard<std::mutex> enq(S.enq);
  ensure_stage_events(ivf, S);
  const uint32_t step = wide ? wide_sub_batch(ivf, R.B, np) : sub_batch(ivf, R.B, R.k, np);
  for (uint32_t o = 0; o < R.B; o += step) {
    const IvfSearch r = R.slice(o, std::min(step, R.B - o), ivf->d, np);
    const float* qpad = nullptr;
    rc = padded_queries(ivf, E, r.q_dev, r.B, &qpad);
    if (rc) return rc;
    HIPCHK(ctx, S.s_probes.ensure((size_t)r.B * np * 4));
    const uint32_t* probes = S.s_probes.as<uint32_t>();
    if (all) {
      hipLaunchKernelGGL(probes_all_kernel, dim3(cdiv((uint64_t)r.B * np, 256)), dim3(256), 0, ctx->stream, r.B, np,
                         S.s_probes.as<uint32_t>());
      mark(ivf, E, EV_COARSE_DONE);
    } else if (r.given_probes) {
      probes = r.given_probes;
      mark(ivf, E, EV_COARSE_BEGIN);
      mark(ivf, E, EV_COARSE_SCANNED);
      mark(ivf, E, EV_COARSE_DONE);
    } else {
      rc = run_coarse(ivf, E, qpad, r.B, np, r.probes_out ? r.probes_out : S.s_probes.as<uint32_t>(), nullptr);
      if (rc) return rc;
    }
    if (R.kind == IvfSearch::COARSE_ONLY) continue;
    const Batch b{qpad, probes, r.B, r.k, np, r.ids, r.dist, r.counts, r.keys, r.given_thr};
    rc = wide ? run_fine_wide(ivf, E, b) : run_fine(ivf, E, b, all ? ROLE_ALL : ROLE_LIST);
    if (rc) return rc;
    rc = finish_profile(ivf, E, !all, true);
    if (rc) return rc;
  }
  ivf->last_set.store(E.S);
  ivf->last_ctx.store(E.ctx);
  return FVDB_OK;
}

int slot_env(fvdb_ivf* ivf, fvdb_ctx* on, uint32_t slot, Env* E) {
  if (slot >= fvdb_ivf::kSlots) FAIL(ivf->ctx, FVDB_E_INVALID, "slot out of range");
  if (on && on->device != ivf->ctx->device) FAIL(ivf->ctx, FVDB_E_INVALID, "context of another device");
  E->ctx = on ? on : ivf->ctx;
  E->S = &slot_scratch(ivf, slot);
  return FVDB_OK;
}
int mask_env(fvdb_ivf* ivf, fvdb_ctx* on, uint32_t slot, fvdb_mask* mask, Env* E) {
  if (!ivf) return FVDB_E_INVALID;
  int rc = slot_env(ivf, on, slot, E);
  if (rc) return rc;
  if (!mask || mask->ivf != ivf) FAIL(ivf->ctx, FVDB_E_INVALID, "mask of another index");
  if (mask->stamp != ivf->mutations) FAIL(ivf->ctx, FVDB_E_INVALID, "stale mask: the index changed after the mask was created");
  E->live = mask->words.as<uint64_t>();
  return FVDB_OK;
}
int slot_done(fvdb_ivf* ivf, const Env& E, int rc) {
  if (rc && E.ctx != ivf->ctx) {
    std::string m;
    {
      std::lock_guard<std::mutex> lk(E.ctx->err_mu);
      m = E.ctx->err;
    }
    ivf->ctx->set_err(m);
  }
  return rc;
}

struct SlotMask {
  bool required = false;
  fvdb_mask* mask = nullptr;
};
constexpr SlotMask kNoMask{};
inline SlotMask masked_by(fvdb_mask* mask) { return SlotMask{true, mask}; }

template <class Body>
int on_slot(fvdb_ivf* ivf, fvdb_ctx* on, uint32_t slot, SlotMask m, Body body) {
  Env E{};
  int rc = m.required ? mask_env(ivf, on, slot, m.mask, &E) : slot_env(ivf, on, slot, &E);
  if (rc) return rc;
  return slot_done(ivf, E, body(E));
}
inline int search_on_slot(fvdb_ivf* ivf, fvdb_ctx* on, uint32_t slot, SlotMask m, const IvfSearch& R) {
  return on_slot(ivf, on, slot, m, [&](const Env& E) { return ivf_search(ivf, E, R); });
}

struct Lease {
  fvdb_ivf* ivf;
  int idx = -1;
  Env E{};
  int rc = FVDB_OK;
  explicit Lease(fvdb_ivf* ivf_) : ivf(ivf_) {
    if (ivf->ctx->profiling) {
      E = Env{ivf->ctx, ivf};
      return;
    }
    std::unique_lock<std::mutex> lk(ivf->mu);
    ivf->lease_cv.wait(lk, [&] { return ivf->lease_busy != (1u << fvdb_ivf::kLeases) - 1u; });
    for (uint32_t i = 0; i < fvdb_ivf::kLeases; ++i)
      if (!(ivf->lease_busy & (1u << i))) {
        idx = (int)i;
        break;
      }
    ivf->lease_busy |= 1u << idx;
    if (!ivf->lease_ctx[idx]) {
      rc = fvdb_ctx_create(ivf->ctx->device, &ivf->lease_ctx[idx]);
      if (rc) ivf->ctx->set_err("could not create a stream for a concurrent search");
    }
    E = Env{ivf->lease_ctx[idx], &ivf->lease_set[idx]};
  }
  ~Lease() {
    if (idx < 0) return;
    {
      std::lock_guard<std::mutex> lk(ivf->mu);
      ivf->lease_busy &= ~(1u << idx);
    }
    ivf->lease_cv.notify_one();
  }
};
template <class Body>
int on_lease(fvdb_ivf* ivf, Body body) {
  Lease L(ivf);
  if (L.rc) return L.rc;
  return slot_done(ivf, L.E, body(L.E));
}
}
}

int fvdb_ivf_search_dev(fvdb_ivf* ivf, const float* q_dev, uint32_t B, uint32_t k, uint32_t nprobe,
                        uint64_t* out_ids_dev, float* out_dist_dev, uint32_t* out_counts_dev, uint64_t* out_keys_dev) {
  return ivf_search(ivf, Env{ivf->ctx, ivf},
                    IvfSearch{IvfSearch::PROBED, q_dev, B, k, nprobe, out_ids_dev, out_dist_dev, out_counts_dev, out_keys_dev});
}

int fvdb_ivf_search_all_dev(fvdb_ivf* ivf, const float* q_dev, uint32_t B, uint32_t k, uint64_t* out_ids_dev,
                            float* out_dist_dev, uint32_t* out_counts_dev) {
  return ivf_search(ivf, Env{ivf->ctx, ivf}, IvfSearch{IvfSearch::ALL, q_dev, B, k, 0, out_ids_dev, out_dist_dev, out_counts_dev});
}

int fvdb_ivf_coarse_dev_slot(fvdb_ivf* ivf, fvdb_ctx* on, uint32_t slot, const float* q_dev, uint32_t B, uint32_t nprobe,
                             uint32_t* out_probes_dev) {
  if (!out_probes_dev) FAIL(ivf->ctx, FVDB_E_INVALID, "null output");
  IvfSearch R{IvfSearch::COARSE_ONLY, q_dev, B, 1, nprobe};
  R.probes_out = out_probes_dev;
  return search_on_slot(ivf, on, slot, kNoMask, R);
}

int fvdb_ivf_search_dev_slot(fvdb_ivf* ivf, fvdb_ctx* on, uint32_t slot, const float* q_dev, uint32_t B, uint32_t k,
                             uint32_t nprobe, uint64_t* out_ids_dev, float* out_dist_dev, uint32_t* out_counts_dev,
                             uint64_t* out_keys_dev) {
  return search_on_slot(ivf, on, slot, kNoMask,
                        IvfSearch{IvfSearch::PROBED, q_dev, B, k, nprobe, out_ids_dev, out_dist_dev, out_counts_dev, out_keys_dev});
}

int fvdb_ivf_search_probes_dev_slot(fvdb_ivf* ivf, fvdb_ctx* on, uint32_t slot, const float* q_dev,
                                    const uint32_t* probes_dev, uint32_t B, uint32_t k, uint32_t nprobe,
                                    uint64_t* out_ids_dev, float* out_dist_dev, uint32_t* out_counts_dev,
                                    uint64_t* out_keys_dev) {
  if (!probes_dev) FAIL(ivf->ctx, FVDB_E_INVALID, "null probes");
  return search_on_slot(ivf, on, slot, kNoMask,
                        IvfSearch{IvfSearch::PROBED, q_dev, B, k, nprobe, out_ids_dev, out_dist_dev, out_counts_dev, out_keys_dev,
                                  probes_dev});
}

int fvdb_ivf_search_dev_slot_masked(fvdb_ivf* ivf, fvdb_ctx* on, uint32_t slot, fvdb_mask* mask, const float* q_dev, uint32_t B,
                                    uint32_t k, uint32_t nprobe, uint64_t* out_ids_dev, float* out_dist_dev,
                                    uint32_t* out_counts_dev, uint64_t* out_keys_dev) {
  return search_on_slot(ivf, on, slot, masked_by(mask),
                        IvfSearch{IvfSearch::PROBED, q_dev, B, k, nprobe, out_ids_dev, out_dist_dev, out_counts_dev, out_keys_dev});
}

int fvdb_ivf_search_probes_dev_slot_masked(fvdb_ivf* ivf, fvdb_ctx* on, uint32_t slot, fvdb_mask* mask, const float* q_dev,
                                           const uint32_t* probes_dev, uint32_t B, uint32_t k, uint32_t nprobe,
                                           uint64_t* out_ids_dev, float* out_dist_dev, uint32_t* out_counts_dev,
                                           uint64_t* out_keys_dev) {
  return on_slot(ivf, on, slot, masked_by(mask), [&](const Env& E) -> int {
    if (!probes_dev) FAIL(E.ctx, FVDB_E_INVALID, "null probes");
    return ivf_search(ivf, E,
                      IvfSearch{IvfSearch::PROBED, q_dev, B, k, nprobe, out_ids_dev, out_dist_dev, out_counts_dev, out_keys_dev,
                                probes_dev});
  });
}

int fvdb_ivf_search_wide_dev_slot(fvdb_ivf* ivf, fvdb_ctx* on, uint32_t slot, fvdb_mask* mask, const float* q_dev, uint32_t B,
                                  uint32_t k, uint32_t nprobe, uint64_t* out_ids_dev, float* out_dist_dev,
                                  uint32_t* out_counts_dev, uint64_t* out_keys_dev) {
  if (!ivf) return FVDB_E_INVALID;
  return search_on_slot(ivf, on, slot, mask ? masked_by(mask) : kNoMask,
                        IvfSearch{IvfSearch::WIDE, q_dev, B, k, nprobe, out_ids_dev, out_dist_dev, out_counts_dev, out_keys_dev});
}

int fvdb_ivf_search_quality_dev(fvdb_ivf* ivf, fvdb_ctx* on, uint32_t slot, const float* q_dev, uint32_t B, uint32_t k,
                                uint32_t nprobe, float* out_recall_dev, float* out_precision_dev) {
  if (!ivf) return FVDB_E_INVALID;
  if (!q_dev || !out_recall_dev || !out_precision_dev) FAIL(ivf->ctx, FVDB_E_INVALID, "null buffer");
  return on_slot(ivf, on, slot, kNoMask, [&](const Env& E) -> int {
    fvdb_ctx* ctx = E.ctx;
    IvfScratch& S = *E.S;
    if (!ivf->trained) FAIL(ctx, FVDB_E_NOT_TRAINED, "index not trained");
    const IvfSearch::Kind kind = k > FVDB_MAX_K ? IvfSearch::WIDE : IvfSearch::PROBED;
    int rc = check_k(ctx, kind, k, probed_lists(ivf, kind, nprobe));
    if (rc) return rc;
    if (B == 0) return FVDB_OK;
    HIPCHK(ctx, hipSetDevice(ctx->device));
    const size_t n = (size_t)B * k;
    HIPCHK(ctx, S.s_qual.ensure(2 * (n * 12 + (size_t)B * 4)));
    char* p = (char*)S.s_qual.p;
    uint64_t* ids[2] = {(uint64_t*)p, (uint64_t*)p + n};
    float* dist[2] = {(float*)(p + n * 16), (float*)(p + n * 16) + n};
    uint32_t* cnt[2] = {(uint32_t*)(p + n * 24), (uint32_t*)(p + n * 24) + B};
    const uint32_t probes[2] = {nprobe, ivf->nlist};
    for (int i = 0; i < 2; ++i) {
      rc = ivf_search(ivf, E, IvfSearch{kind, q_dev, B, k, probes[i], ids[i], dist[i], cnt[i]});
      if (rc) return rc;
    }
    hipLaunchKernelGGL(search_quality_kernel, dim3(cdiv(B, 4)), dim3(256), 0, ctx->stream, ids[0], cnt[0], ids[1], cnt[1], B, k,
                       out_recall_dev, out_precision_dev);
    HIPCHK(ctx, hipGetLastError());
    return FVDB_OK;
  });
}

static int search_host(fvdb_ivf* ivf, IvfSearch::Kind kind, const float* q, uint32_t B, uint32_t k, uint32_t nprobe,
                       uint64_t* out_ids, float* out_dist, uint32_t* out_counts) {
  if (!ivf->trained) FAIL(ivf->ctx, FVDB_E_NOT_TRAINED, "index not trained");
  if (B == 0) return FVDB_OK;
  int rc = check_k(ivf->ctx, kind, k, probed_lists(ivf, kind, nprobe));
  if (rc) return rc;
  rc = check_finite(ivf->ctx, q, (uint64_t)B * ivf->d);
  if (rc) return rc;
  return on_lease(ivf, [&](const Env& E) -> int {
    fvdb_ctx* ctx = E.ctx;
    IvfScratch& S = *E.S;
    HIPCHK(ctx, hipSetDevice(ctx->device));
    HIPCHK(ctx, S.s_in.ensure((size_t)B * ivf->d * 4));
// ... 724 lines not shown
```

fabstir-vectordb_amd/host/fvdb_host.hpp:

```cpp
#pragma once
#include <atomic>
#include <condition_variable>
#include <cstdint>
#include <memory>
#include <mutex>
#include <shared_mutex>
#include <string>
#include <unordered_map>
#include <unordered_set>
#include <vector>

#include "../../include/fvdb.h"

namespace fvdbh {

struct SplitMix64 {
  uint64_t s;
  explicit SplitMix64(uint64_t seed) : s(seed) {}
  uint64_t next() {
    uint64_t z = (s += 0x9E3779B97F4A7C15ull);
    z = (z ^ (z >> 30)) * 0xBF58476D1CE4E5B9ull;
    z = (z ^ (z >> 27)) * 0x94D049BB133111EBull;
    return z ^ (z >> 31);
  }
// ... 19 lines not shown

struct Visited {
  std::vector<uint32_t> keys, stamp;
  uint32_t epoch = 0, used = 0;
  void reset(size_t expect);
  bool insert(uint32_t v);
 private:
  void grow();
};

inline void fill_empty(uint64_t* ids, float* dist, uint32_t* counts, uint32_t B, uint32_t k) {
  for (uint32_t b = 0; b < B; ++b) counts[b] = 0;
  for (size_t i = 0; i < (size_t)B * k; ++i) {
    ids[i] = FVDB_NO_ID;
    dist[i] = __builtin_huge_valf();
  }
}

struct DevBuf {
  fvdb_ctx* ctx = nullptr;
  void *dev = nullptr, *host = nullptr;
  uint64_t cap = 0;
  int reserve(fvdb_ctx* c, uint64_t bytes, bool pinned) {
    if (bytes <= cap) return FVDB_OK;
    release();
    ctx = c;
    if (fvdb_dev_alloc(c, bytes, &dev) || (pinned && fvdb_host_alloc(c, bytes, &host))) return FVDB_E_OOM;
    cap = bytes;
    return FVDB_OK;
  }
  void release() {
    if (dev) fvdb_dev_free(ctx, dev);
    if (host) fvdb_host_free(ctx, host);
    dev = host = nullptr;
    cap = 0;
  }
};

typedef std::shared_ptr<fvdb_mask> MaskRef;
inline MaskRef adopt_mask(fvdb_mask* m) { return MaskRef(m, [](fvdb_mask* p) { fvdb_mask_destroy(p); }); }
inline bool mask_fresh(const MaskRef& m) {
  fvdb_mask_info_t info;
  return m && fvdb_mask_info(m.get(), &info) == FVDB_OK && !info.stale;
}

inline int slot_ctx(fvdb_ctx* base, bool borrow, fvdb_ctx** ctx) {
  if (*ctx) return FVDB_OK;
  if (!borrow) return fvdb_ctx_create(fvdb_ctx_device(base), ctx);
  *ctx = base;
  return FVDB_OK;
}

struct IVFConfig {
  uint32_t n_clusters = 256, n_probe = 16, train_size = 10000, max_iterations = 25;
  uint64_t seed = 0;
  bool is_valid() const { return n_clusters > 0 && n_probe > 0 && n_probe <= n_clusters && train_size > 0 && max_iterations > 0; }
};

class IVFIndex {
 public:
  IVFIndex(fvdb_ctx* ctx, const IVFConfig& cfg);
  ~IVFIndex();
  const IVFConfig& config() const { return cfg_; }
  bool is_trained() const { return trained_; }
  uint32_t dimension() const { return dim_; }
  uint64_t total_vectors() const { return total_; }
  int train(const float* data, uint64_t n, uint32_t dim, fvdb_train_result* out);
  int set_trained(const float* centroids, uint32_t dim);
  int get_centroids(float* out) const;
  int insert(uint64_t id, const float* v, uint32_t dim);
  int batch_insert(const uint64_t* ids, const float* v, uint64_t n, uint32_t dim, uint64_t* n_ok, int* first_error);
  int batch_insert_assigned(const uint64_t* ids, const float* v, uint64_t n, uint32_t dim, const uint32_t* clusters,
                            uint64_t* n_ok, int* first_error);
  int batch_insert_from_store(const uint64_t* ids, fvdb_store* store, const uint32_t* rows, uint64_t n, uint64_t* n_ok,
                              int* first_error);
  int assign(const float* v, uint64_t n, uint32_t dim, uint32_t* out);
  int get_vector_by_id(uint64_t id, float* out);
  int get_vectors(const uint64_t* ids, uint64_t n, float* out, uint8_t* found);
  int find_cluster(const float* v, uint32_t dim, uint32_t* out);
  int search(const float* q, uint32_t B, uint32_t dim, uint32_t k, uint32_t n_probe, uint64_t* ids, float* dist,
             uint32_t* counts);
  int search_dev(const float* q_dev, uint32_t B, uint32_t dim, uint32_t k, uint32_t n_probe, uint64_t* ids_dev,
                 float* dist_dev, uint32_t* counts_dev, fvdb_ctx* on = nullptr, uint32_t slot = 0);
  int search_allowed(const float* q, uint32_t B, uint32_t dim, uint32_t k, uint32_t n_probe, const uint64_t* allowed,
                     uint64_t n_allowed, uint64_t* ids, float* dist, uint32_t* counts);
  int allowed_mask(const uint64_t* allowed, uint64_t n_allowed, MaskRef* out);
  int search_dev_masked(const MaskRef& mask, const float* q_dev, uint32_t B, uint32_t dim, uint32_t k, uint32_t n_probe,
                        uint64_t* ids_dev, float* dist_dev, uint32_t* counts_dev, fvdb_ctx* on = nullptr, uint32_t slot = 0);
  uint64_t mask_builds() const { return mask_builds_; }
  int mark_deleted(uint64_t id);
  bool is_deleted(uint64_t id) const { return deleted_.count(id) > 0; }
  uint64_t active_count() const { return total_ - deleted_.size(); }
  uint64_t deleted_count() const { return deleted_.size(); }
  int vacuum(uint64_t* removed);
  struct RetrainResult {
    uint64_t old_clusters, new_clusters, vectors_reassigned, converged;
  };
  struct ClusterStats {
    uint64_t n_clusters, total_vectors, empty_clusters;
    float avg_cluster_size, size_variance;
  };
  int retrain(const IVFConfig& new_config, RetrainResult* out);
  int add_clusters(uint32_t n_clusters_to_add, uint64_t* vectors_reassigned);
  int optimize_clusters(uint32_t* iterations, float* improvement);
  ClusterStats get_cluster_stats() const;
  struct SearchQuality {
    float avg_recall, avg_precision, avg_query_time_ms;
    uint64_t queries_evaluated;
  };
  int evaluate_search_quality(const float* q, uint32_t B, uint32_t dim, uint32_t k, SearchQuality* out);
  uint64_t cluster_size(uint32_t c) const;
  int export_list(uint32_t c, float* rows, uint64_t* ids, uint8_t* live) const;
  void clear_lists();
  fvdb_ivf* device() { return dev_; }

 private:
  struct Loc {
    uint32_t cluster, pos;
  };
  int ensure_device(uint32_t dim);
  float size_variance() const;
  int rebuild(uint32_t n_clusters, uint32_t max_iterations, uint64_t seed, fvdb_train_result* tr, uint64_t* reinserted);
  int place(const uint64_t* ids, const float* v, uint64_t n, const uint32_t* clusters, uint64_t* n_ok, int* first_error);
  std::vector<uint64_t> accept(const uint64_t* ids, uint64_t n, const uint32_t* clusters, int* first_error);
  fvdb_ctx* ctx_;
  IVFConfig cfg_;
  fvdb_ivf* dev_ = nullptr;
  uint32_t dev_clusters_ = 0;
  uint32_t dim_ = 0;
  bool trained_ = false;
  bool live_again_ = false;
  uint64_t total_ = 0;
  std::unordered_multimap<uint64_t, Loc> where_;
  std::unordered_set<uint64_t> deleted_;
  std::mutex mask_mu_;
  std::vector<uint64_t> mask_key_;
  MaskRef mask_;
  uint64_t mask_builds_ = 0;
  std::mutex allowed_mu_;
  DevBuf allowed_q_, allowed_out_;
  void drop_mask() {
    mask_.reset();
    mask_key_.clear();
  }
};

struct HNSWConfig {
  uint32_t max_connections = 16, max_connections_layer_0 = 32, ef_construction = 200;
  uint64_t seed = 0;
};

class HNSWIndex {
 public:
  struct AllowView {
    MaskRef mask;
    std::vector<uint8_t> eff;
    uint64_t allowed_live = 0;
  };
  typedef std::shared_ptr<const AllowView> ViewRef;
  HNSWIndex(fvdb_ctx* ctx, const HNSWConfig& cfg);
  ~HNSWIndex();
  const HNSWConfig& config() const { return cfg_; }
  uint64_t node_count() const { return n_registered_; }
  bool entry_point(uint64_t* id) const;
  uint32_t dimension() const { return dim_; }
  size_t assign_level();
// ... 218 lines not shown
                         uint64_t* ids, float* dist, uint32_t* counts);
  int search_allowed(const float* q, uint32_t B, uint32_t dim, const HybridSearchConfig& cfg, const uint64_t* allowed,
                     uint64_t n_allowed, double now, uint64_t* ids, float* dist, uint32_t* counts);
  void set_blocking_writers(bool on) { writers_wait_ = on; }
  bool blocking_writers() const { return writers_wait_; }
  bool busy() const {
    std::lock_guard<std::mutex> lk(slot_mu_);
    for (const Slot& s : slots_)
      if (s.active) return true;
    return false;
  }
  bool migration_due(double threshold_s, double now) const {
    return !pending_migration_.empty() && age_of(now, pending_min_ts_) >= threshold_s;
  }
  uint64_t migrate_with_threshold(double threshold_s, double now);
  void set_resident_migration(bool on) { resident_migration_ = on; }
  bool resident_migration() const { return resident_migration_; }
  enum MigrationPath : int { MIGRATION_NONE = 0, MIGRATION_RESIDENT = 1, MIGRATION_HOST = 2 };
  int migration_info(fvdb_maintenance_info_t* out) const {
    *out = migration_info_;
    return migration_path_;
  }
  int get_vectors(const uint64_t* ids, uint64_t n, float* out, uint8_t* found);
  int remove(uint64_t id, double now);
  uint64_t recent_count() const { return recent_count_; }
  uint64_t historical_count() const { return historical_count_; }
  int from_parts(const uint64_t* ids, const double* ts, uint64_t n, uint64_t recent_count, uint64_t historical_count,
                 bool ivf_trained);
  int vacuum(uint64_t* hnsw_removed, uint64_t* ivf_removed);
  int retrain_historical(const IVFConfig& new_ivf_config, IVFIndex::RetrainResult* out);
  uint64_t timestamp_count() const { return ts_order_.size(); }
  void export_timestamps(uint64_t* ids, double* ts) const;
  HNSWIndex& recent() { return *recent_; }
  IVFIndex& historical() { return *historical_; }
  void set_sequential_graph(bool on) { sequential_graph_ = on; }
  bool sequential_graph() const { return sequential_graph_; }
  double recent_build_seconds() const { return recent_build_s_; }
  int bulk_insert(const uint64_t* ids, const float* v, uint64_t n, uint32_t dim, const double* ts, double now);
  int bulk_insert_sharded(const uint64_t* ids, const float* v, uint64_t n, uint32_t dim, const double* ts, double now,
                          uint32_t rank, uint32_t world, uint32_t* owner_out );

 private:
  static double age_of(double now, double ts) { return now - ts < 0 ? 0.0 : now - ts; }
  int search_impl(const float* q, bool q_on_device, uint32_t B, uint32_t dim, const HybridSearchConfig& cfg,
                  double now, uint64_t* ids, float* dist, uint32_t* counts, const uint64_t* allowed = nullptr,
                  uint64_t n_allowed = 0, bool masked = false);
  int begin_explicit(uint32_t slot, const float* q_dev, uint32_t B, uint32_t dim, const HybridSearchConfig& cfg,
                     int shard_mode, double now);
  int begin_impl(uint32_t slot, const float* q_dev, uint32_t B, uint32_t dim, const HybridSearchConfig& cfg,
                 int shard_mode = -1);
  int migrate_if_due(double now, bool in_flight_before);
  struct Slice {
    uint32_t per, lo, hi;
  };
  Slice strong_slice(uint32_t B) const;
  int build_recent(const uint64_t* ids, const float* v, uint64_t n, uint32_t dim);
  int bulk_route(const uint64_t* ids, const float* v, uint64_t n, uint32_t dim, const double* ts, double now,
                 std::vector<uint64_t>& hid, std::vector<float>& hv);
  bool sequential_graph_ = true;
  bool resident_migration_ = true;
  int migration_path_ = MIGRATION_NONE;
  fvdb_maintenance_info_t migration_info_{};
  std::atomic<bool> writers_wait_{false};
  int write_lock(std::unique_lock<std::shared_mutex>& w);
  double recent_build_s_ = 0.0;
  fvdb_comm* comm_ = nullptr;
  fvdb_sharded* sharded_ = nullptr;
  uint32_t shard_rank_ = 0, shard_world_ = 0;
  std::vector<uint32_t> shard_owner_;
  std::vector<uint64_t> shard_sizes_;
  uint64_t migrate_locked(double threshold_s, double now);
  bool busy_unlocked() const {
    for (const Slot& s : slots_)
      if (s.active) return true;
    return false;
  }
  mutable std::shared_mutex rw_;
  mutable std::mutex slot_mu_;
  std::condition_variable slot_cv_;
  fvdb_ctx* ctx_ivf_;
  struct Slot {
    DevBuf ivf;
    uint32_t ivf_rows = 0;
    fvdb_event* ivf_done = nullptr;
    fvdb_ctx* ivf_ctx = nullptr;
    bool active = false, ivf_in_flight = false, hnsw_in_flight = false, recent = false;
    DevBuf d_q;
    const float* q = nullptr;
    uint32_t B = 0, dim = 0, k = 0, rk = 0, hk = 0, ef = 0;
    MaskRef ivf_mask;
    HNSWIndex::ViewRef view;
  };
  Slot slots_[kSlots];
  struct Lease {
    static constexpr uint32_t kAnyFree = ~0u;
    enum How { kTake, kAdopt };
    Lease(HybridIndex* h, uint32_t slot, How how);
    ~Lease();
    Lease(const Lease&) = delete;
    Lease& operator=(const Lease&) = delete;
    void hand_over() { sl = nullptr; }
    uint32_t index() const { return (uint32_t)(sl - h->slots_); }
    HybridIndex* h;
    Slot* sl = nullptr;
  };
  HybridConfig cfg_;
  HNSWIndex* recent_;
  IVFIndex* historical_;
  bool initialized_ = false, ivf_trained_ = false;
  std::vector<uint64_t> ts_order_;
  std::unordered_map<uint64_t, double> timestamps_;
  struct Pending {
    uint64_t id;
    double ts;
  };
  std::vector<Pending> pending_migration_;
  double pending_min_ts_ = 1e300;
  uint64_t recent_count_ = 0, historical_count_ = 0;
};

void plan_list_owners_host(const uint64_t* sizes, uint32_t nlist, uint32_t world, uint32_t* owner);
void merge_parts_host(uint32_t B, uint32_t k, uint32_t rk, uint32_t hk, const uint64_t* rid, const float* rd,
                      const uint32_t* rc, const uint64_t* hid, const float* hd, const uint32_t* hc, uint64_t* ids,
                      float* dist, uint32_t* counts);

}
```

fabstir-vectordb_amd/host/hybrid_index.cpp:

```cpp
#include <algorithm>
#include <chrono>
#include <cmath>
#include <cstdio>
#include <cstdlib>
#include <cstring>

#include "fvdb_host.hpp"

namespace fvdbh {

HybridIndex::HybridIndex(fvdb_ctx* ctx_ivf, fvdb_ctx* ctx_hnsw, const HybridConfig& cfg) : ctx_ivf_(ctx_ivf), cfg_(cfg) {
  recent_ = new HNSWIndex(ctx_hnsw, cfg.hnsw);
  historical_ = new IVFIndex(ctx_ivf, cfg.ivf);
}

HybridIndex::~HybridIndex() {
  for (Slot& sl : slots_) {
    sl.ivf.release();
    if (sl.ivf_done) fvdb_event_destroy(sl.ivf_done);
    sl.d_q.release();
    if (sl.ivf_ctx && sl.ivf_ctx != ctx_ivf_) fvdb_ctx_destroy(sl.ivf_ctx);
  }
  if (sharded_) fvdb_sharded_destroy(sharded_);
  delete recent_;
// ... 432 lines not shown
int HybridIndex::migrate_if_due(double now, bool in_flight_before) {
  if (!cfg_.auto_migrate) return FVDB_OK;
  {
    std::shared_lock<std::shared_mutex> r(rw_);
    if (!migration_due(cfg_.recent_threshold_s, now)) return FVDB_OK;
  }
  std::unique_lock<std::shared_mutex> w(rw_);
  if (!migration_due(cfg_.recent_threshold_s, now)) return FVDB_OK;
  if (in_flight_before || busy()) return FVDB_E_INVALID;
  migrate_locked(cfg_.recent_threshold_s, now);
  return FVDB_OK;
}

int HybridIndex::search_dev_begin(uint32_t slot, const float* q_dev, uint32_t B, uint32_t dim, const HybridSearchConfig& cfg,
                                  double now) {
  if (slot >= kSlots) return FVDB_E_INVALID;
  return begin_explicit(slot, q_dev, B, dim, cfg, -1, now);
}

int HybridIndex::begin_explicit(uint32_t slot, const float* q_dev, uint32_t B, uint32_t dim, const HybridSearchConfig& cfg,
                                int shard_mode, double now) {
  bool others = false;
  {
    std::lock_guard<std::mutex> lk(slot_mu_);
    if (slots_[slot].active) return FVDB_E_INVALID;
    others = busy_unlocked();
  }
  if (initialized_ && cfg.k != 0 && (B != 0 || shard_mode >= 0))
    if (int rc = migrate_if_due(now, others)) return rc;
  std::shared_lock<std::shared_mutex> r(rw_);
  Lease lease(this, slot, Lease::kTake);
  if (!lease.sl) return FVDB_E_INVALID;
  lease.hand_over();
  slots_[slot].ivf_mask.reset();
  slots_[slot].view.reset();
  return begin_impl(slot, q_dev, B, dim, cfg, shard_mode);
}

int HybridIndex::attach_comm(fvdb_comm* comm) {
  std::unique_lock<std::shared_mutex> w(rw_);
  if (busy()) return FVDB_E_INVALID;
  if (sharded_) fvdb_sharded_destroy(sharded_);
  sharded_ = nullptr;
  comm_ = comm;
  if (!comm) return FVDB_OK;
  if (!ivf_trained_ || !historical_->device()) return FVDB_E_NOT_TRAINED;
  return fvdb_sharded_create(historical_->device(), comm, &sharded_);
}

HybridIndex::Slice HybridIndex::strong_slice(uint32_t B) const {
  const uint32_t W = (uint32_t)fvdb_comm_world(comm_), r = (uint32_t)fvdb_comm_rank(comm_);
  const uint32_t per = (B + W - 1) / W;
  return {per, std::min(B, r * per), std::min(B, (r + 1) * per)};
}

uint32_t HybridIndex::sharded_rows(uint32_t B, int mode) const {
  if (!comm_ || mode != FVDB_SHARD_STRONG) return B;
  const Slice s = strong_slice(B);
  return s.hi - s.lo;
}

int HybridIndex::search_sharded_begin(uint32_t slot, const float* q_dev, uint32_t B, uint32_t dim,
                                      const HybridSearchConfig& cfg, int mode, double now) {
  if (slot >= kSlots || !sharded_ || (mode != FVDB_SHARD_WEAK && mode != FVDB_SHARD_STRONG)) return FVDB_E_INVALID;
  return begin_explicit(slot, q_dev, B, dim, cfg, mode, now);
}

namespace {
struct IvfBlock {
  uint64_t* ids = nullptr;
  float* dist = nullptr;
  uint32_t* counts = nullptr;
  static uint64_t bytes(uint32_t rows, uint32_t hk) { return (uint64_t)rows * hk * 12 + (uint64_t)rows * 4; }
  IvfBlock() = default;
  IvfBlock(void* base, uint32_t rows, uint32_t hk) {
    const uint64_t need = (uint64_t)rows * hk;
    ids = (uint64_t*)base;
    dist = (float*)((char*)base + need * 8);
    counts = (uint32_t*)((char*)base + need * 12);
  }
};
}

int HybridIndex::begin_impl(uint32_t slot, const float* q_dev, uint32_t B, uint32_t dim, const HybridSearchConfig& cfg,
                            int shard_mode) {
  Slot& sl = slots_[slot];
  sl.ivf_in_flight = sl.hnsw_in_flight = false;
  const float* q_own = q_dev;
  uint32_t Bown = B, ivf_rows = B;
  if (shard_mode == FVDB_SHARD_STRONG) {
    const Slice s = strong_slice(B);
    q_own = q_dev + (size_t)s.lo * dim;
    Bown = s.hi - s.lo;
    ivf_rows = s.per;
  }
  const uint32_t B_ivf_in = B;
  B = Bown;
  sl.q = q_own;
  sl.B = B;
  sl.dim = dim;
  sl.k = (uint32_t)cfg.k;
  sl.rk = (uint32_t)(cfg.recent_k > 0 ? cfg.recent_k : cfg.k);
  sl.hk = (uint32_t)(cfg.historical_k > 0 ? cfg.historical_k : cfg.k);
  sl.ef = (uint32_t)cfg.hnsw_ef;
  sl.recent = cfg.search_recent;
  if (!initialized_ || sl.k == 0 || (B == 0 && shard_mode < 0)) return FVDB_OK;
  if (cfg.search_recent && B > 0) {
    int rcb = 0;
    sl.hnsw_in_flight = recent_->search_dev_begin(q_own, B, dim, sl.rk, sl.ef, &rcb, slot, sl.view.get());
  }
  if (cfg.search_historical && ivf_trained_) {
    const uint64_t bytes = IvfBlock::bytes(ivf_rows, sl.hk);
    if (int rc = sl.ivf.reserve(ctx_ivf_, bytes, true)) return rc;
    sl.ivf_rows = ivf_rows;
    const IvfBlock d(sl.ivf.dev, ivf_rows, sl.hk);
    static const bool one_stream = getenv("FVDB_IVF_ONE_STREAM") != nullptr;
    if (slot_ctx(ctx_ivf_, slot == 0 || one_stream, &sl.ivf_ctx)) return FVDB_E_HIP;
    fvdb_ctx* on = sl.ivf_ctx == ctx_ivf_ ? nullptr : sl.ivf_ctx;
    if (!sl.ivf_done && fvdb_event_create(sl.ivf_ctx, &sl.ivf_done)) return FVDB_E_HIP;
    if (shard_mode >= 0) {
      if (dim != historical_->dimension()) return FVDB_E_DIM;
      const int rcs = fvdb_ivf_search_sharded_begin(sharded_, on, on ? slot : 0, q_dev, B_ivf_in, sl.hk,
                                                    (uint32_t)cfg.ivf_n_probe, shard_mode, d.ids, d.dist, d.counts);
      if (rcs) return rcs;
      sl.ivf_in_flight = true;
    } else {
      const int rch = sl.ivf_mask ? historical_->search_dev_masked(sl.ivf_mask, q_dev, B, dim, sl.hk, (uint32_t)cfg.ivf_n_probe,
                                                                   d.ids, d.dist, d.counts, on, on ? slot : 0)
                                  : historical_->search_dev(q_dev, B, dim, sl.hk, (uint32_t)cfg.ivf_n_probe, d.ids, d.dist,
                                                            d.counts, on, on ? slot : 0);
      if (rch) return rch;
      sl.ivf_in_flight = true;
    }
    if (sl.ivf_in_flight) {
      if (fvdb_dev_download_async(sl.ivf_ctx, sl.ivf.host, sl.ivf.dev, (size_t)bytes) || fvdb_event_record(sl.ivf_ctx, sl.ivf_done))
        return FVDB_E_HIP;
    }
  }
  return FVDB_OK;
}

int HybridIndex::search_dev_end(uint32_t slot, uint64_t* ids, float* dist, uint32_t* counts) {
  if (slot >= kSlots) return FVDB_E_INVALID;
  Lease lease(this, slot, Lease::kAdopt);
  if (!lease.sl) return FVDB_E_INVALID;
  Slot& sl = *lease.sl;
  const uint32_t B = sl.B, k = sl.k;
  struct DropMasks {
    Slot& sl;
    ~DropMasks() {
      sl.ivf_mask.reset();
      sl.view.reset();
    }
  } drop_masks{sl};
  fill_empty(ids, dist, counts, B, k);
  if (!initialized_ || B == 0 || k == 0) return FVDB_OK;
  std::vector<uint64_t> rid;
  std::vector<float> rd;
  std::vector<uint32_t> rc_(B, 0);
  bool have_r = false, have_h = false;
  if (sl.recent) {
    rid.resize((size_t)B * sl.rk);
    rd.resize((size_t)B * sl.rk);
    int rc2;
    if (sl.hnsw_in_flight) {
      rc2 = recent_->search_dev_end(sl.q, B, sl.dim, sl.rk, sl.ef, rid.data(), rd.data(), rc_.data(), slot, sl.view.get());
    } else if (sl.view) {
      rc2 = recent_->search_dev_view(sl.q, B, sl.dim, sl.rk, sl.ef, *sl.view, rid.data(), rd.data(), rc_.data());
    } else {
      rc2 = recent_->search_dev(sl.q, B, sl.dim, sl.rk, sl.ef, rid.data(), rd.data(), rc_.data());
    }
    have_r = rc2 == FVDB_OK;
  }
  IvfBlock h;
  if (sl.ivf_in_flight) {
    have_h = fvdb_event_wait(sl.ivf_ctx, sl.ivf_done) == FVDB_OK;
    h = IvfBlock(sl.ivf.host, sl.ivf_rows, sl.hk);
    bool others = false;
    {
      std::lock_guard<std::mutex> lk(slot_mu_);
      for (const Slot& o : slots_) others = others || (o.active && &o != &sl);
    }
    if (!others) fvdb_ivf_profile_collect(historical_->device());
  }
  merge_parts(B, k, sl.rk, sl.hk, have_r, rid.data(), rd.data(), rc_.data(), have_h, h.ids, h.dist, h.counts, ids, dist,
              counts);
  return FVDB_OK;
}

int HybridIndex::search_impl(const float* q, bool q_on_device, uint32_t B, uint32_t dim, const HybridSearchConfig& cfg,
                             double now, uint64_t* ids, float* dist, uint32_t* counts, const uint64_t* allowed,
                             uint64_t n_allowed, bool masked) {
  const uint32_t k = (uint32_t)cfg.k;
  fill_empty(ids, dist, counts, B, k);
  if (!initialized_ || B == 0 || k == 0) return FVDB_OK;
  if (int rc = migrate_if_due(now, false)) return rc;
  std::shared_lock<std::shared_mutex> r(rw_);
  MaskRef ivf_mask;
  HNSWIndex::ViewRef view;
  if (masked) {
    if (cfg.search_recent)
      if (int rc = recent_->allowed_view(allowed, n_allowed, &view)) return rc;
    if (cfg.search_historical && ivf_trained_)
      if (int rc = historical_->allowed_mask(allowed, n_allowed, &ivf_mask)) return rc;
  }
  Lease lease(this, Lease::kAnyFree, Lease::kTake);
  Slot& sl = *lease.sl;
  const uint32_t slot = lease.index();
  sl.ivf_mask = ivf_mask;
  sl.view = view;
  struct DropMasks {
    Slot* sl;
    ~DropMasks() {
      if (!sl) return;
      sl->ivf_mask.reset();
      sl->view.reset();
    }
  } drop_masks{&sl};
  const float* qd = q;
  if (!q_on_device) {
    const uint64_t bytes = (uint64_t)B * dim * 4;
    if (int rc = sl.d_q.reserve(ctx_ivf_, bytes, false)) return rc;
    if (slot_ctx(ctx_ivf_, slot == 0, &sl.ivf_ctx)) return FVDB_E_HIP;
    for (uint64_t i = 0; i < (uint64_t)B * dim; ++i)
      if (!(q[i] - q[i] == 0.0f)) return FVDB_E_NONFINITE;
    const int rcu = fvdb_dev_upload(sl.ivf_ctx, sl.d_q.dev, q, bytes);
    if (rcu) return rcu;
    qd = (const float*)sl.d_q.dev;
  }
  const int rc0 = begin_impl(slot, qd, B, dim, cfg);
// ... 61 lines not shown
```

fabstir-vectordb_amd/host/ivf_index.cpp:

```cpp
#include <algorithm>
#include <chrono>
#include <cstring>

#include "fvdb_host.hpp"

namespace fvdbh {

IVFIndex::IVFIndex(fvdb_ctx* ctx, const IVFConfig& cfg) : ctx_(ctx), cfg_(cfg) {}

IVFIndex::~IVFIndex() {
  drop_mask();
  allowed_q_.release();
  allowed_out_.release();
  if (dev_) fvdb_ivf_destroy(dev_);
}

int IVFIndex::ensure_device(uint32_t dim) {
  if (dev_ && dim_ == dim && dev_clusters_ == cfg_.n_clusters) return FVDB_OK;
  if (dev_) {
    drop_mask();
    fvdb_ivf_destroy(dev_);
    dev_ = nullptr;
  }
  int rc = fvdb_ivf_create(ctx_, dim, cfg_.n_clusters, &dev_);
// ... 335 lines not shown
    found[i] = 1;
    cl.push_back(best.cluster);
    ps.push_back(best.pos);
    at.push_back(i);
  }
  if (at.empty()) return FVDB_OK;
  if (!dev_) return FVDB_E_NOT_TRAINED;
  if (at.size() == n) return fvdb_ivf_get_rows(dev_, cl.data(), ps.data(), n, out);
  std::vector<float> rows(at.size() * (size_t)dim_);
  const int rc = fvdb_ivf_get_rows(dev_, cl.data(), ps.data(), at.size(), rows.data());
  if (rc) {
    for (uint64_t i : at) found[i] = 0;
    return rc;
  }
  for (size_t j = 0; j < at.size(); ++j) std::memcpy(out + at[j] * dim_, &rows[j * dim_], dim_ * sizeof(float));
  return FVDB_OK;
}

int IVFIndex::get_vector_by_id(uint64_t id, float* out) {
  uint8_t found = 0;
  const int rc = get_vectors(&id, 1, out, &found);
  return rc ? rc : (found ? FVDB_OK : FVDB_E_NOT_FOUND);
}

int IVFIndex::insert(uint64_t id, const float* v, uint32_t dim) {
  if (!trained_) return FVDB_E_NOT_TRAINED;
  if (dim != dim_) return FVDB_E_DIM;
  uint32_t c = 0;
  int rc = fvdb_ivf_assign(dev_, v, 1, &c);
  if (rc) return rc;
  uint64_t ok = 0;
  int err = 0;
  rc = place(&id, v, 1, &c, &ok, &err);
  if (rc) return rc;
  return ok == 1 ? FVDB_OK : err;
}

int IVFIndex::batch_insert(const uint64_t* ids, const float* v, uint64_t n, uint32_t dim, uint64_t* n_ok,
                           int* first_error) {
  if (n_ok) *n_ok = 0;
  if (first_error) *first_error = 0;
  if (!trained_) return FVDB_E_NOT_TRAINED;
  if (dim != dim_) return FVDB_E_DIM;
  if (n == 0) return FVDB_OK;
  std::vector<uint32_t> clusters(n);
  int rc = fvdb_ivf_assign(dev_, v, n, clusters.data());
  if (rc) return rc;
  return place(ids, v, n, clusters.data(), n_ok, first_error);
}

int IVFIndex::batch_insert_assigned(const uint64_t* ids, const float* v, uint64_t n, uint32_t dim,
                                    const uint32_t* clusters, uint64_t* n_ok, int* first_error) {
  if (n_ok) *n_ok = 0;
  if (first_error) *first_error = 0;
  if (!trained_) return FVDB_E_NOT_TRAINED;
  if (dim != dim_) return FVDB_E_DIM;
  if (n == 0) return FVDB_OK;
  return place(ids, v, n, clusters, n_ok, first_error);
}

int IVFIndex::assign(const float* v, uint64_t n, uint32_t dim, uint32_t* out) {
  if (!trained_) return FVDB_E_NOT_TRAINED;
  if (dim != dim_) return FVDB_E_DIM;
  return fvdb_ivf_assign(dev_, v, n, out);
}

int IVFIndex::search(const float* q, uint32_t B, uint32_t dim, uint32_t k, uint32_t n_probe, uint64_t* ids,
                     float* dist, uint32_t* counts) {
  if (!trained_) return FVDB_E_NOT_TRAINED;
  if (dim != dim_) return FVDB_E_DIM;
  if (k > FVDB_MAX_K) return fvdb_ivf_search_wide(dev_, q, B, k, n_probe, ids, dist, counts);
  return fvdb_ivf_search(dev_, q, B, k, n_probe, ids, dist, counts);
}

int IVFIndex::search_dev(const float* q_dev, uint32_t B, uint32_t dim, uint32_t k, uint32_t n_probe, uint64_t* ids_dev,
                         float* dist_dev, uint32_t* counts_dev, fvdb_ctx* on, uint32_t slot) {
  if (!trained_) return FVDB_E_NOT_TRAINED;
  if (dim != dim_) return FVDB_E_DIM;
  if (k > FVDB_MAX_K)
    return fvdb_ivf_search_wide_dev_slot(dev_, on, slot, nullptr, q_dev, B, k, n_probe, ids_dev, dist_dev, counts_dev, nullptr);
  return fvdb_ivf_search_dev_slot(dev_, on, slot, q_dev, B, k, n_probe, ids_dev, dist_dev, counts_dev, nullptr);
}

int IVFIndex::allowed_mask(const uint64_t* allowed, uint64_t n_allowed, MaskRef* out) {
  if (!trained_ || !dev_) return FVDB_E_NOT_TRAINED;
  if (n_allowed && !allowed) return FVDB_E_INVALID;
  std::lock_guard<std::mutex> lk(mask_mu_);
  const bool same = mask_ && mask_key_.size() == n_allowed &&
                    (n_allowed == 0 || std::memcmp(mask_key_.data(), allowed, n_allowed * 8) == 0);
  if (!same || !mask_fresh(mask_)) {
    drop_mask();
    fvdb_mask* m = nullptr;
    const int rc = fvdb_mask_create_ivf(dev_, allowed, n_allowed, &m);
    if (rc) return rc;
    mask_ = adopt_mask(m);
    mask_key_.assign(allowed, allowed + n_allowed);
    mask_builds_ += 1;
  }
  *out = mask_;
  return FVDB_OK;
}

int IVFIndex::search_dev_masked(const MaskRef& mask, const float* q_dev, uint32_t B, uint32_t dim, uint32_t k, uint32_t n_probe,
                                uint64_t* ids_dev, float* dist_dev, uint32_t* counts_dev, fvdb_ctx* on, uint32_t slot) {
  if (!trained_) return FVDB_E_NOT_TRAINED;
  if (dim != dim_) return FVDB_E_DIM;
  if (k > FVDB_MAX_K)
    return fvdb_ivf_search_wide_dev_slot(dev_, on, slot, mask.get(), q_dev, B, k, n_probe, ids_dev, dist_dev, counts_dev, nullptr);
  return fvdb_ivf_search_dev_slot_masked(dev_, on, slot, mask.get(), q_dev, B, k, n_probe, ids_dev, dist_dev, counts_dev, nullptr);
}

int IVFIndex::search_allowed(const float* q, uint32_t B, uint32_t dim, uint32_t k, uint32_t n_probe, const uint64_t* allowed,
                             uint64_t n_allowed, uint64_t* ids, float* dist, uint32_t* counts) {
  if (!trained_) return FVDB_E_NOT_TRAINED;
  if (dim != dim_) return FVDB_E_DIM;
  if (B == 0) return FVDB_OK;
  if (k == 0 || k > FVDB_MAX_K_WIDE) return FVDB_E_UNSUPPORTED;
  for (uint64_t i = 0; i < (uint64_t)B * dim; ++i)
    if (!(q[i] - q[i] == 0.0f)) return FVDB_E_NONFINITE;
  MaskRef mask;
  int rc = allowed_mask(allowed, n_allowed, &mask);
  if (rc) return rc;
  std::lock_guard<std::mutex> lk(allowed_mu_);
  const uint64_t need = (uint64_t)B * k, bytes = need * 12 + (uint64_t)B * 4;
  if ((rc = allowed_q_.reserve(ctx_, (uint64_t)B * dim * 4, false)) || (rc = allowed_out_.reserve(ctx_, bytes, true))) return rc;
  if ((rc = fvdb_dev_upload(ctx_, allowed_q_.dev, q, (size_t)B * dim * 4))) return rc;
  char* d = (char*)allowed_out_.dev;
  rc = search_dev_masked(mask, (const float*)allowed_q_.dev, B, dim, k, n_probe, (uint64_t*)d, (float*)(d + need * 8),
                         (uint32_t*)(d + need * 12));
  if (rc) return rc;
  if ((rc = fvdb_dev_download_async(ctx_, allowed_out_.host, allowed_out_.dev, (size_t)bytes)) || (rc = fvdb_ctx_synchronize(ctx_)))
    return rc;
  const char* h = (const char*)allowed_out_.host;
  std::memcpy(ids, h, need * 8);
  std::memcpy(dist, h + need * 8, need * 4);
  std::memcpy(counts, h + need * 12, (size_t)B * 4);
  return FVDB_OK;
}

int IVFIndex::mark_deleted(uint64_t id) {
  auto r = where_.equal_range(id);
  if (r.first == r.second) return FVDB_E_NOT_FOUND;
  deleted_.insert(id);
  std::vector<uint32_t> cl, ps;
  for (auto it = r.first; it != r.second; ++it) {
    cl.push_back(it->second.cluster);
    ps.push_back(it->second.pos);
  }
  return fvdb_ivf_set_deleted(dev_, cl.data(), ps.data(), cl.size(), 1);
}

}
```

include/fvdb.h:

```cpp
#ifndef FVDB_H
#define FVDB_H

#include <stddef.h>
#include <stdint.h>

#ifdef __cplusplus
extern "C" {
#endif

typedef enum fvdb_status {
  FVDB_OK = 0,
  FVDB_E_NOT_TRAINED = 1,
  FVDB_E_DUPLICATE = 2,
  FVDB_E_DIM = 3,
  FVDB_E_INSUFFICIENT = 4,
  FVDB_E_INCONSISTENT = 5,
  FVDB_E_INVALID = 6,
  FVDB_E_NOT_FOUND = 7,
  FVDB_E_NOT_INITIALIZED = 8,
  FVDB_E_NONFINITE = 9,
  FVDB_E_HIP = 10,
  FVDB_E_OOM = 11,
  FVDB_E_UNSUPPORTED = 12,
  FVDB_E_RCCL = 13
// ... 17 lines not shown
  int device, compute_units, hw_queues, hw_queues_source;
} fvdb_ctx_info_t;
int fvdb_ctx_info(fvdb_ctx* ctx, fvdb_ctx_info_t* out);
void* fvdb_ctx_stream(fvdb_ctx* ctx);
const char* fvdb_last_error(fvdb_ctx* ctx);
const char* fvdb_version(void);
int fvdb_dev_alloc(fvdb_ctx* ctx, size_t bytes, void** out);
int fvdb_dev_free(fvdb_ctx* ctx, void* p);
int fvdb_dev_upload(fvdb_ctx* ctx, void* dst_dev, const void* src_host, size_t bytes);
int fvdb_dev_download(fvdb_ctx* ctx, void* dst_host, const void* src_dev, size_t bytes);
int fvdb_host_alloc(fvdb_ctx* ctx, size_t bytes, void** out);
void fvdb_host_free(fvdb_ctx* ctx, void* p);
int fvdb_dev_download_async(fvdb_ctx* ctx, void* dst_pinned, const void* src_dev, size_t bytes);
typedef struct fvdb_event fvdb_event;
int fvdb_event_create(fvdb_ctx* ctx, fvdb_event** out);
void fvdb_event_destroy(fvdb_event* e);
int fvdb_event_record(fvdb_ctx* ctx, fvdb_event* e);
int fvdb_event_wait(fvdb_ctx* ctx, fvdb_event* e);
int fvdb_timer_start(fvdb_ctx* ctx);
int fvdb_timer_stop_ms(fvdb_ctx* ctx, float* out_ms);
int fvdb_ctx_set_profiling(fvdb_ctx* ctx, int on);

int fvdb_dot_products(fvdb_ctx* ctx, const float* q, uint32_t B, const float* x, uint64_t n, uint32_t d, float* out);
int fvdb_cosine_similarities(fvdb_ctx* ctx, const float* q, uint32_t B, const float* x, uint64_t n, uint32_t d,
                             float* out);

int fvdb_ivf_create(fvdb_ctx* ctx, uint32_t d, uint32_t nlist, fvdb_ivf** out);
typedef enum fvdb_dtype { FVDB_F32 = 0, FVDB_F16 = 1 } fvdb_dtype;
int fvdb_ivf_create_ex(fvdb_ctx* ctx, uint32_t d, uint32_t nlist, int row_dtype, fvdb_ivf** out);
void fvdb_ivf_destroy(fvdb_ivf* ivf);
int fvdb_ivf_set_centroids(fvdb_ivf* ivf, const float* centroids);
int fvdb_ivf_get_centroids(fvdb_ivf* ivf, float* out );
typedef struct fvdb_train_result {
  uint32_t iterations;
  uint32_t converged;
  float initial_error;
  float final_error;
} fvdb_train_result;
int fvdb_ivf_train(fvdb_ivf* ivf, const float* x, uint64_t n, uint32_t max_iterations, uint64_t seed,
                   fvdb_train_result* out);
int fvdb_ivf_assign(fvdb_ivf* ivf, const float* x, uint64_t n, uint32_t* out_cluster);
int fvdb_ivf_add(fvdb_ivf* ivf, const float* x, const uint64_t* ids, uint64_t n, uint32_t* out_cluster,
                 uint32_t* out_pos);
int fvdb_ivf_add_assigned(fvdb_ivf* ivf, const float* x, const uint64_t* ids, uint64_t n,
                          const uint32_t* cluster, uint32_t* out_pos);
int fvdb_ivf_set_deleted(fvdb_ivf* ivf, const uint32_t* cluster, const uint32_t* pos, uint64_t n, int deleted);
int fvdb_ivf_list_sizes(fvdb_ivf* ivf, uint64_t* out );
uint64_t fvdb_ivf_total_rows(fvdb_ivf* ivf);
int fvdb_ivf_list_export(fvdb_ivf* ivf, uint32_t list, float* rows, uint64_t* ids, uint8_t* live);
int fvdb_ivf_reserve(fvdb_ivf* ivf, uint64_t n_rows);

typedef struct fvdb_maintenance_info_t {
  uint64_t rows_in, rows_out;
  uint64_t host_bytes;
  uint64_t move_bytes;
  float ms_gather, ms_train, ms_assign, ms_ranks, ms_move;
  float ms_total;
} fvdb_maintenance_info_t;
int fvdb_ivf_compact(fvdb_ivf* ivf, uint64_t* removed, uint64_t* out_ids);
int fvdb_ivf_train_from(fvdb_ivf* dst, fvdb_ivf* src, uint32_t max_iterations, uint64_t seed, fvdb_train_result* out);
int fvdb_ivf_assign_from(fvdb_ivf* dst, fvdb_ivf* src, uint32_t* out_cluster, uint64_t* out_ids);
int fvdb_ivf_refill_from(fvdb_ivf* dst, fvdb_ivf* src, uint64_t n_rows, uint32_t* out_pos);
int fvdb_ivf_maintenance_info(fvdb_ivf* ivf, fvdb_maintenance_info_t* out);

int fvdb_ivf_get_rows(fvdb_ivf* ivf, const uint32_t* cluster, const uint32_t* pos, uint64_t n, float* out_rows );
int fvdb_ivf_get_rows_dev(fvdb_ivf* ivf, fvdb_ctx* on, const uint32_t* cluster, const uint32_t* pos, uint64_t n,
                          float* out_rows_dev);
int fvdb_ivf_assign_from_store(fvdb_ivf* ivf, fvdb_store* store, const uint32_t* rows, uint64_t n, uint32_t* out_cluster);
int fvdb_ivf_add_assigned_from_store(fvdb_ivf* ivf, fvdb_store* store, const uint32_t* rows, const uint64_t* ids,
                                     uint64_t n, const uint32_t* cluster, uint32_t* out_pos);
int fvdb_ivf_clear(fvdb_ivf* ivf);
int fvdb_ivf_set_global_list_sizes(fvdb_ivf* ivf, const uint64_t* sizes );

int fvdb_ivf_search(fvdb_ivf* ivf, const float* q, uint32_t B, uint32_t k, uint32_t nprobe, uint64_t* out_ids,
                    float* out_dist, uint32_t* out_counts);
int fvdb_ivf_search_dev(fvdb_ivf* ivf, const float* q_dev, uint32_t B, uint32_t k, uint32_t nprobe,
                        uint64_t* out_ids_dev, float* out_dist_dev, uint32_t* out_counts_dev,
                        uint64_t* out_keys_dev);
int fvdb_ivf_search_all(fvdb_ivf* ivf, const float* q, uint32_t B, uint32_t k, uint64_t* out_ids,
                        float* out_dist, uint32_t* out_counts);
int fvdb_ivf_search_dev_slot(fvdb_ivf* ivf, fvdb_ctx* on, uint32_t slot, const float* q_dev, uint32_t B, uint32_t k,
                             uint32_t nprobe, uint64_t* out_ids_dev, float* out_dist_dev, uint32_t* out_counts_dev,
                             uint64_t* out_keys_dev);
int fvdb_ivf_coarse_dev_slot(fvdb_ivf* ivf, fvdb_ctx* on, uint32_t slot, const float* q_dev, uint32_t B, uint32_t nprobe,
                             uint32_t* out_probes_dev);
int fvdb_ivf_search_probes_dev_slot(fvdb_ivf* ivf, fvdb_ctx* on, uint32_t slot, const float* q_dev,
                                    const uint32_t* probes_dev, uint32_t B, uint32_t k, uint32_t nprobe,
                                    uint64_t* out_ids_dev, float* out_dist_dev, uint32_t* out_counts_dev,
                                    uint64_t* out_keys_dev);
int fvdb_ivf_search_all_dev(fvdb_ivf* ivf, const float* q_dev, uint32_t B, uint32_t k, uint64_t* out_ids_dev,
                            float* out_dist_dev, uint32_t* out_counts_dev);
int fvdb_ivf_coarse(fvdb_ivf* ivf, const float* q, uint32_t B, uint32_t nprobe, uint32_t* out_clusters,
                    float* out_dist);

#define FVDB_COARSE_AUTO 0
#define FVDB_COARSE_EXACT 1
int fvdb_ivf_set_coarse_mode(fvdb_ivf* ivf, int mode);
int fvdb_ivf_coarse_fallbacks(fvdb_ivf* ivf, uint64_t* out);

#define FVDB_SCAN_AUTO 0
#define FVDB_SCAN_EXACT 1
#define FVDB_SCAN_FILTER 2
int fvdb_ivf_set_scan_mode(fvdb_ivf* ivf, int mode);
int fvdb_ivf_scan_fallbacks(fvdb_ivf* ivf, uint64_t* out);
int fvdb_ivf_scan_fallback_reasons(fvdb_ivf* ivf, uint64_t* out5);

int fvdb_ivf_scan_survivors(fvdb_ivf* ivf, uint32_t* out, uint32_t B);

int fvdb_ivf_scan_survivor_dump(fvdb_ivf* ivf, uint32_t query, uint32_t max_n, uint32_t* rank, uint32_t* pos, float* v,
                                uint32_t* n_out);

typedef struct fvdb_search_stats {
  uint64_t rows_scanned;
  uint64_t work_items;
  uint64_t list_rows_touched;
} fvdb_search_stats;
int fvdb_ivf_last_stats(fvdb_ivf* ivf, fvdb_search_stats* out);
uint64_t fvdb_ivf_stage_times(fvdb_ivf* ivf, float* ms_out);
int fvdb_ivf_profile_collect(fvdb_ivf* ivf);

int fvdb_merge_keys_dev(fvdb_ctx* ctx, const uint64_t* keys_dev, const uint64_t* ids_dev, uint32_t G, uint32_t B,
                        uint32_t k, uint64_t* out_ids_dev, float* out_dist_dev, uint32_t* out_counts_dev);

int fvdb_top_k_indices(fvdb_ctx* ctx, const float* scores , uint32_t B, uint64_t n, uint32_t k,
                       uint64_t* out_idx, uint32_t* out_counts);
int fvdb_top_k_indices_heap(fvdb_ctx* ctx, const float* scores, uint32_t B, uint64_t n, uint32_t k, uint64_t* out_idx,
                            uint32_t* out_counts);
int fvdb_top_k_indices_dev(fvdb_ctx* ctx, const float* scores_dev, uint32_t B, uint64_t n, uint32_t k, int heap,
                           uint64_t* out_idx_dev, uint32_t* out_counts_dev);
int fvdb_streaming_top_k(fvdb_ctx* ctx, const uint64_t* ids, const float* scores, uint32_t B, uint64_t n, uint32_t k,
                         uint64_t* out_ids, float* out_scores, uint32_t* out_counts);
int fvdb_streaming_top_k_dev(fvdb_ctx* ctx, const uint64_t* ids_dev, const float* scores_dev, uint32_t B, uint64_t n,
                             uint32_t k, uint64_t* out_ids_dev, float* out_scores_dev, uint32_t* out_counts_dev);
int fvdb_merge_search_results(fvdb_ctx* ctx, const uint64_t* ids, const float* dist, uint32_t B, uint64_t n, uint32_t k,
                              uint64_t* out_ids, float* out_dist, uint32_t* out_counts);
int fvdb_merge_search_results_dev(fvdb_ctx* ctx, const uint64_t* ids_dev, const float* dist_dev, uint32_t B, uint64_t n,
                                  uint32_t k, uint64_t* out_ids_dev, float* out_dist_dev, uint32_t* out_counts_dev);

int fvdb_store_create(fvdb_ctx* ctx, uint32_t d, uint64_t capacity_rows, fvdb_store** out);
void fvdb_store_destroy(fvdb_store* s);
int fvdb_store_append(fvdb_store* s, const float* rows, uint64_t n, uint64_t* first_row);
uint64_t fvdb_store_rows(fvdb_store* s);
int fvdb_store_get(fvdb_store* s, uint64_t row, float* out );
int fvdb_score_candidates(fvdb_store* s, const float* q, uint32_t B, const uint32_t* cand, uint32_t C, float* out);
typedef struct fvdb_scorer fvdb_scorer;
int fvdb_scorer_create(fvdb_store* s, uint32_t max_B, uint32_t max_C, fvdb_scorer** out);
void fvdb_scorer_destroy(fvdb_scorer* sc);
int fvdb_scorer_set_queries(fvdb_scorer* sc, const float* q, uint32_t B);
int fvdb_scorer_set_query_rows(fvdb_scorer* sc, const uint32_t* rows, uint32_t B);
int fvdb_scorer_set_queries_dev(fvdb_scorer* sc, const float* q_dev, uint32_t B);
uint32_t* fvdb_scorer_cand_buffer(fvdb_scorer* sc);
const float* fvdb_scorer_dist_buffer(fvdb_scorer* sc);
int fvdb_scorer_run(fvdb_scorer* sc, uint32_t B, uint32_t C);
int fvdb_scorer_launch(fvdb_scorer* sc, uint32_t B, uint32_t C);
int fvdb_scorer_wait(fvdb_scorer* sc);

typedef struct fvdb_graph fvdb_graph;
int fvdb_graph_create(fvdb_store* s, fvdb_graph** out);
void fvdb_graph_destroy(fvdb_graph* g);
int fvdb_graph_upload(fvdb_graph* g, uint32_t n, const uint32_t* levels, const uint8_t* deleted,
                      const uint32_t* slot_start, const uint32_t* adj, uint32_t entry_node);
int fvdb_graph_set_deleted(fvdb_graph* g, uint32_t node, int deleted);
int fvdb_graph_search_dev(fvdb_graph* g, const float* q_dev, uint32_t B, uint32_t k, uint32_t ef,
                          uint32_t* out_nodes_dev, float* out_dist_dev, uint32_t* out_counts_dev,
                          uint32_t* out_status_dev);
int fvdb_graph_search_dev_slot(fvdb_graph* g, fvdb_ctx* on, uint32_t slot, const float* q_dev, uint32_t B, uint32_t k,
// ... 108 lines not shown
```

Baseline: 1.788 million.

## Pair concurrent IVF search batches into one shared MFMA filter pass

Splits the MFMA fine scan into a front stage (query prep and threshold) and a back stage (filter, refine, verify). A batch whose front has finished can wait so the next slot's batch joins it, and both run through one combined filter launch over shared query rows, synchronised with cross-stream events. The aim is fewer, larger filter launches that keep the GPU busier. The cost is extra latency for the waiting batch, more complex event handling across streams, and skipping refine on deferred batches, which could affect recall. Pairing is controlled by a knob (FVDB_IVF_PAIR defaults to 0, plus a pairing field initialised to -1).

```diff
diff --git a/fabstir-vectordb_amd/_capi.py b/fabstir-vectordb_amd/_capi.py
--- a/fabstir-vectordb_amd/_capi.py
+++ b/fabstir-vectordb_amd/_capi.py
@@ -129,6 +129,10 @@
     "fvdb_ctx_device": (i32, [vp]),
     "fvdb_ctx_info": (i32, [vp, vp]),
     "fvdb_ivf_search_dev_slot": (i32, [vp, vp, u32, vp, u32, u32, u32, vp, vp, vp, vp]),
+    "fvdb_ivf_search_begin_dev_slot": (i32, [vp, vp, u32, vp, u32, u32, u32, vp, vp, vp, i32, C.POINTER(i32)]),
+    "fvdb_ivf_search_flush_slot": (i32, [vp, u32]),
+    "fvdb_ivf_pair_stats": (i32, [vp, u64p, u64p]),
+    "fvdb_ivf_set_pairing": (i32, [vp, i32]),
     "fvdb_ivf_coarse_dev_slot": (i32, [vp, vp, u32, vp, u32, u32, vp]),
     "fvdb_ivf_search_probes_dev_slot": (i32, [vp, vp, u32, vp, vp, u32, u32, u32, vp, vp, vp, vp]),
     "fvdb_host_alloc": (i32, [vp, C.c_size_t, C.POINTER(vp)]),
diff --git a/fabstir-vectordb_amd/csrc/fvdb_hip.cpp b/fabstir-vectordb_amd/csrc/fvdb_hip.cpp
--- a/fabstir-vectordb_amd/csrc/fvdb_hip.cpp
+++ b/fabstir-vectordb_amd/csrc/fvdb_hip.cpp
@@ -146,8 +146,28 @@
 };
 constexpr size_t kScalarsBytes = 64;
 
+struct Batch {
+  const float* qpad;
+  const uint32_t* probes;
+  uint32_t B, k, np;
+  uint64_t* out_ids;
+  float* out_dist;
+  uint32_t* out_counts;
+  uint64_t* out_keys;
+  const float* given_thr = nullptr;
+};
+
 struct IvfScratch {
   std::mutex enq;
+  struct Front {
+    bool live = false;
+    fvdb_ctx* ctx = nullptr;
+    Batch b{};
+    uint32_t rows = 0;
+    uint64_t stamp = 0;
+  } front;
+  hipEvent_t front_done = nullptr, filter_done = nullptr, guest_done = nullptr;
+  bool guest = false;
   bool pend_filter = false;
   bool pending_profile = false, pend_coarse = false, pend_fine = false, collecting = false;
   std::vector<DBuf*> bufs;
@@ -171,6 +191,12 @@
     for (DBuf* b : bufs) b->release();
     if (fetch_done) (void)hipEventDestroy(fetch_done);
     fetch_done = nullptr;
+    for (hipEvent_t* e : {&front_done, &filter_done, &guest_done}) {
+      if (*e) (void)hipEventDestroy(*e);
+      *e = nullptr;
+    }
+    front = Front{};
+    guest = false;
     for (auto& e : sev) {
       if (e) (void)hipEventDestroy(e);
       e = nullptr;
@@ -209,6 +235,8 @@
   uint32_t backoff_len = 0;
   uint64_t overflow_seen = 0, overflow_q = 0;
   uint32_t refine_batches_left = 0;
+  std::atomic<uint64_t> paired_batches{0}, solo_batches{0};
+  std::atomic<int> pairing{-1};
   DBuf d_mfma_stamps;
   int mfma_stamps_launch = 0;
   DBuf d_xmax;
@@ -243,6 +271,8 @@
   fvdb_ctx* ctx;
   IvfScratch* S;
   const uint64_t* live = nullptr;
+  IvfScratch* Q = nullptr;
+  uint32_t qo = 0;
 };
 inline IvfScratch& slot_scratch(fvdb_ivf* ivf, uint32_t slot) { return slot == 0 ? *ivf : ivf->spare[slot - 1]; }
 inline const uint64_t* live_words(const fvdb_ivf* ivf, const Env& E) { return E.live ? E.live : ivf->pool.valid; }
@@ -279,6 +309,7 @@
   bool mfma_threshold_pass = has("FVDB_MFMA_THRESHOLD_PASS");
   uint32_t mfma_segb_a = (uint32_t)std::max(1, num("FVDB_MFMA_SEGB_A", 1));
   bool mfma_no_refine = has("FVDB_MFMA_NO_REFINE");
+  bool pair = num("FVDB_IVF_PAIR", 0) != 0;
 #ifdef FVDB_MFMA_STAMPS_BUILD
   int mfma_stamps = num("FVDB_MFMA_STAMPS", 0);
 #endif
@@ -393,17 +424,6 @@
 inline void mark(const fvdb_ivf* ivf, const Env& E, StageEvent e) {
   if (ivf->ctx->profiling) (void)hipEventRecord(E.S->sev[e], E.ctx->stream);
 }
-
-struct Batch {
-  const float* qpad;
-  const uint32_t* probes;
-  uint32_t B, k, np;
-  uint64_t* out_ids;
-  float* out_dist;
-  uint32_t* out_counts;
-  uint64_t* out_keys;
-  const float* given_thr = nullptr;
-};
 
 inline ListTable list_table(const fvdb_ivf* ivf) {
   return ListTable{ivf->t_off.as<uint32_t>(), ivf->t_blocks.as<uint32_t>(), ivf->nlist};
@@ -577,7 +597,7 @@
   fvdb_ctx* ctx = E.ctx;
   IvfScratch& S = *E.S;
   const uint32_t nlist = ivf->nlist;
-  HIPCHK(ctx, S.s_cnt.ensure((size_t)nlist * 4));
+  HIPCHK(ctx, S.s_cnt.ensure((size_t)(nlist + 2) * 4));
   HIPCHK(ctx, S.s_fill.ensure((size_t)nlist * 4));
   HIPCHK(ctx, S.s_eoff.ensure((size_t)(nlist + 1) * 4));
   HIPCHK(ctx, S.s_ioff.ensure((size_t)(nlist + 1) * 4));
@@ -621,6 +641,23 @@
 }
 inline bool half_rows(const fvdb_ivf* ivf) { return ivf->f16 || ivf->pool.half != nullptr; }
 inline int x_rounded(const fvdb_ivf* ivf) { return ivf->f16 ? 0 : (ivf->pool.half ? 1 : 2); }
+
+struct QueryRows {
+  _Float16* qh;
+  float *qn2, *thr;
+  uint32_t *scnt, *mslots;
+  u32x2* surv;
+  float* sval;
+};
+inline QueryRows query_rows(const fvdb_ivf* ivf, const Env& E) {
+  const IvfScratch& Q = E.Q ? *E.Q : *E.S;
+  const size_t o = E.qo;
+  return QueryRows{(_Float16*)Q.s_qh.p + o * ivf->dpad, Q.s_qn2.as<float>() + o,      Q.s_thr.as<float>() + o,
+                   Q.s_scnt.as<uint32_t>() + o,          Q.s_mslots.as<uint32_t>() + o * 64,
+                   (u32x2*)Q.s_surv.p + o * kMfmaCmax,   Q.s_sdist.as<float>() + o * kMfmaCmax};
+}
+inline uint32_t* batch_words(const fvdb_ivf* ivf, const Env& E) { return E.S->s_cnt.as<uint32_t>() + ivf->nlist; }
+inline uint32_t pair_rows(uint32_t B) { return std::min<uint32_t>(std::max<uint32_t>(2 * B, 256u), 16384u); }
 
 struct MfmaPlan {
   bool wg;
@@ -666,36 +703,37 @@
   return FVDB_OK;
 }
 
-int mfma_scratch(fvdb_ivf* ivf, const Env& E, const MfmaPlan& P, uint32_t B, uint32_t np) {
+int mfma_scratch(fvdb_ivf* ivf, const Env& E, const MfmaPlan& P, uint32_t B, uint32_t np, uint32_t rows) {
   fvdb_ctx* ctx = E.ctx;
   IvfScratch& S = *E.S;
-  HIPCHK(ctx, S.s_qh.ensure((size_t)(B + 1) * ivf->dpad * 2));
-  HIPCHK(ctx, S.s_qn2.ensure((size_t)B * 4));
-  HIPCHK(ctx, S.s_thr.ensure((size_t)B * 4));
+  if (!E.Q) {
+    HIPCHK(ctx, S.s_qh.ensure((size_t)(rows + 1) * ivf->dpad * 2));
+    HIPCHK(ctx, S.s_qn2.ensure((size_t)rows * 4));
+    HIPCHK(ctx, S.s_thr.ensure((size_t)rows * 4));
+    HIPCHK(ctx, S.s_mslots.ensure((size_t)rows * 64 * 4));
+    HIPCHK(ctx, S.s_surv.ensure((size_t)rows * P.cmax * 8));
+    HIPCHK(ctx, S.s_sdist.ensure((size_t)rows * P.cmax * 4));
+    HIPCHK(ctx, S.s_scnt.ensure((size_t)(rows + 2) * 4));
+  }
   HIPCHK(ctx, S.s_tA.ensure((size_t)B * 4));
   HIPCHK(ctx, S.s_pa.ensure((size_t)B * 4));
-  HIPCHK(ctx, S.s_mslots.ensure((size_t)B * 64 * 4));
-  HIPCHK(ctx, S.s_surv.ensure((size_t)B * P.cmax * 8));
-  HIPCHK(ctx, S.s_sdist.ensure((size_t)B * P.cmax * 4));
-  HIPCHK(ctx, S.s_scnt.ensure((size_t)(B + 2) * 4));
   HIPCHK(ctx, S.s_fail.ensure((size_t)B * 4));
   HIPCHK(ctx, S.s_part.ensure((size_t)P.fpart * 8));
-  int rc = plan_scratch(ivf, E, B, np);
+  int rc = plan_scratch(ivf, E, E.Q ? B : rows, np);
   if (rc) return rc;
   HIPCHK(ctx, S.s_scalars.ensure(kScalarsBytes));
   return FVDB_OK;
 }
 
 void launch_prep_queries(fvdb_ivf* ivf, const Env& E, const float* qpad, uint32_t B) {
-  IvfScratch& S = *E.S;
-  hipLaunchKernelGGL(prep_queries_kernel, dim3(cdiv(B + 1, 4)), dim3(256), 0, E.ctx->stream, qpad, B, ivf->dpad,
-                     (_Float16*)S.s_qh.p, S.s_qn2.as<float>(), S.s_cnt.as<uint32_t>(), ivf->nlist,
-                     S.s_scnt.as<uint32_t>(), S.s_mslots.as<uint32_t>());
+  const QueryRows r = query_rows(ivf, E);
+  hipLaunchKernelGGL(prep_queries_kernel, dim3(cdiv(B + 1, 4)), dim3(256), 0, E.ctx->stream, qpad, B, ivf->dpad, r.qh, r.qn2,
+                     E.S->s_cnt.as<uint32_t>(), ivf->nlist + 2, r.scnt, r.mslots);
 }
 
 ThresholdArgs threshold_args(fvdb_ivf* ivf, const Env& E, const float* qpad, const uint32_t* probes, uint32_t B,
                              uint32_t k, uint32_t np, float* thr_out) {
-  const IvfScratch& S = *E.S;
+  const QueryRows r = query_rows(ivf, E);
   ThresholdArgs t{};
   t.rows = ivf->pool.half ? ivf->pool.half : ivf->pool.data;
   t.pool_valid = live_words(ivf, E);
@@ -704,9 +742,9 @@
   t.lists = list_table(ivf);
   t.list_len = ivf->t_len.as<uint32_t>();
   t.probes = probes;
-  t.qh = (const _Float16*)S.s_qh.p;
+  t.qh = r.qh;
   t.queries = qpad;
-  t.qn = S.s_qn2.as<float>();
+  t.qn = r.qn2;
   t.xmax_bits = ivf->d_xmax.as<uint32_t>();
   t.B = B;
   t.np = np;
@@ -768,14 +806,15 @@
   hipLaunchKernelGGL(kernel, dim3(P.grid), dim3(256), 0, ctx->stream, a);
 }
 
-void mfma_threshold(fvdb_ivf* ivf, const Env& E, const MfmaPlan& P, const Batch& b, const MfmaScanArgs& a) {
+void mfma_threshold(fvdb_ivf* ivf, const Env& E, const MfmaPlan& P, const Batch& b) {
   fvdb_ctx* ctx = E.ctx;
   IvfScratch& S = *E.S;
   if (b.given_thr) return;
   if (!ivf_knobs().mfma_threshold_pass) {
-    launch_threshold_direct(ivf, ctx, threshold_args(ivf, E, b.qpad, b.probes, b.B, b.k, b.np, S.s_thr.as<float>()));
+    launch_threshold_direct(ivf, ctx, threshold_args(ivf, E, b.qpad, b.probes, b.B, b.k, b.np, query_rows(ivf, E).thr));
     return;
   }
+  const MfmaScanArgs a = mfma_scan_args(ivf, E, P, b);
   hipLaunchKernelGGL(first_probe_kernel, dim3(cdiv(b.B, 256)), dim3(256), 0, ctx->stream, b.probes, b.B, b.np,
                      ivf->t_len.as<uint32_t>(), 256u, S.s_pa.as<uint32_t>());
   launch_plan(ivf, E, S.s_pa.as<uint32_t>(), b.B, 1, P.segbA, P.Q, nullptr, S.s_cnt.as<uint32_t>());
@@ -926,13 +965,14 @@
   v.probes = b.probes;
   v.glob_blocks = ivf->t_glob.as<uint32_t>();
   v.queries = b.qpad;
-  v.qn = S.s_qn2.as<float>();
+  const QueryRows r = query_rows(ivf, E);
+  v.qn = r.qn2;
   v.xmax_bits = ivf->d_xmax.as<uint32_t>();
-  v.thr = b.given_thr ? b.given_thr : S.s_thr.as<float>();
+  v.thr = b.given_thr ? b.given_thr : r.thr;
   v.remote_thr = b.given_thr ? 1 : 0;
-  v.surv = (const u32x2*)S.s_surv.p;
-  v.sval = S.s_sdist.as<float>();
-  v.scnt = S.s_scnt.as<uint32_t>();
+  v.surv = r.surv;
+  v.sval = r.sval;
+  v.scnt = r.scnt;
   v.B = b.B;
   v.k = b.k;
   v.ka = P.ka;
@@ -949,7 +989,7 @@
   v.fallbacks = ivf->fb_word(FB_SCAN, E.live != nullptr);
   v.reasons = ivf->fb_word(FB_REASONS, E.live != nullptr);
   v.fail_list = S.s_fail.as<uint32_t>();
-  v.nfail = S.s_scnt.as<uint32_t>() + b.B;
+  v.nfail = batch_words(ivf, E);
   return v;
 }
 void launch_select(fvdb_ivf* ivf, fvdb_ctx* ctx, const VerifyArgs& v) {
@@ -966,7 +1006,7 @@
   fa.queries = b.qpad;
   fa.fail_list = v.fail_list;
   fa.nfail = v.nfail;
-  fa.head = S.s_scnt.as<uint32_t>() + b.B + 1;
+  fa.head = batch_words(ivf, E) + 1;
   fa.k = b.k;
   fa.nprobe = b.np;
   fa.dpad = ivf->dpad;
@@ -999,24 +1039,18 @@
   return FVDB_OK;
 }
 
-int run_fine_mfma(fvdb_ivf* ivf, const Env& E, const Batch& b) {
-  fvdb_ctx* ctx = E.ctx;
-  const IvfKnobs& kn = ivf_knobs();
-  MfmaPlan P;
-  int rc = mfma_plan(ivf, ctx, kn, b.B, b.k, b.np, &P);
-  if (rc) return rc;
-  rc = mfma_scratch(ivf, E, P, b.B, b.np);
+int mfma_front(fvdb_ivf* ivf, const Env& E, const MfmaPlan& P, const Batch& b, uint32_t rows) {
+  int rc = mfma_scratch(ivf, E, P, b.B, b.np, rows);
   if (rc) return rc;
   mark(ivf, E, EV_SCAN_BEGIN);
   launch_prep_queries(ivf, E, b.qpad, b.B);
-  MfmaScanArgs a = mfma_scan_args(ivf, E, P, b);
-  mfma_threshold(ivf, E, P, b, a);
-  rc = mfma_filter(ivf, E, P, b, &a);
-  if (rc) return rc;
-  if (!b.given_thr && !kn.mfma_no_refine && (ivf->scan_mode != FVDB_SCAN_AUTO || auto_refines(ivf))) {
-    rc = mfma_refine(ivf, E, P, b, a);
-    if (rc) return rc;
-  }
+  mfma_threshold(ivf, E, P, b);
+  HIPCHK(E.ctx, hipGetLastError());
+  return FVDB_OK;
+}
+
+int mfma_finish(fvdb_ivf* ivf, const Env& E, const MfmaPlan& P, const Batch& b) {
+  fvdb_ctx* ctx = E.ctx;
   mark(ivf, E, EV_SCAN_DONE);
   E.S->pend_filter = true;
   const VerifyArgs v = verify_args(ivf, E, P, b);
@@ -1024,21 +1058,57 @@
   mfma_rescan(ivf, E, P, b, v);
   mark(ivf, E, EV_FINE_DONE);
   if (!E.live) {
-    rc = mfma_watch_counters(ivf, ctx, b.B);
+    int rc = mfma_watch_counters(ivf, ctx, b.B);
     if (rc) return rc;
   }
   HIPCHK(ctx, hipGetLastError());
   return FVDB_OK;
 }
 
-int run_fine(fvdb_ivf* ivf, const Env& E, const Batch& b, int role) {
+int mfma_back(fvdb_ivf* ivf, const Env& E, const MfmaPlan& P, const Batch& b, bool refine) {
+  MfmaScanArgs a = mfma_scan_args(ivf, E, P, b);
+  int rc = mfma_filter(ivf, E, P, b, &a);
+  if (rc) return rc;
+  if (refine) {
+    rc = mfma_refine(ivf, E, P, b, a);
+    if (rc) return rc;
+  }
+  return mfma_finish(ivf, E, P, b);
+}
+
+struct FineRoute {
+  bool mfma = false;
+  bool refine = false;
+};
+FineRoute fine_route(fvdb_ivf* ivf, const Env& E, const Batch& b, int role) {
+  FineRoute r;
+  r.mfma = (ivf->scan_mode == FVDB_SCAN_AUTO || ivf->scan_mode == FVDB_SCAN_FILTER) && !ivf_knobs().scan_exact &&
+           mfma_shape_ok(ivf, b.B, b.k, b.np) && role == ROLE_LIST && ivf->pool.norms != nullptr;
+  if (r.mfma && E.live && ivf->scan_mode == FVDB_SCAN_AUTO) r.mfma = false;
+  if (r.mfma && ivf->scan_mode == FVDB_SCAN_AUTO && auto_backs_off(ivf)) r.mfma = false;
+  r.refine = r.mfma && !b.given_thr && !ivf_knobs().mfma_no_refine && (ivf->scan_mode != FVDB_SCAN_AUTO || auto_refines(ivf));
+  return r;
+}
+
+int run_fine(fvdb_ivf* ivf, const Env& E, const Batch& b, int role, const FineRoute& route, bool defer) {
   E.S->pend_filter = false;
-  bool mfma = (ivf->scan_mode == FVDB_SCAN_AUTO || ivf->scan_mode == FVDB_SCAN_FILTER) && !ivf_knobs().scan_exact &&
-              mfma_shape_ok(ivf, b.B, b.k, b.np) && role == ROLE_LIST && ivf->pool.norms != nullptr;
-  if (mfma && E.live && ivf->scan_mode == FVDB_SCAN_AUTO) mfma = false;
-  if (mfma && ivf->scan_mode == FVDB_SCAN_AUTO && auto_backs_off(ivf)) mfma = false;
-  if (mfma) return run_fine_mfma(ivf, E, b);
-  return run_fine_exact(ivf, E, b, role);
+  if (!route.mfma) return run_fine_exact(ivf, E, b, role);
+  MfmaPlan P;
+  int rc = mfma_plan(ivf, E.ctx, ivf_knobs(), b.B, b.k, b.np, &P);
+  if (rc) return rc;
+  const uint32_t rows = defer ? pair_rows(b.B) : b.B;
+  rc = mfma_front(ivf, E, P, b, rows);
+  if (rc) return rc;
+  if (!defer) return mfma_back(ivf, E, P, b, route.refine);
+  IvfScratch& S = *E.S;
+  if (!S.front_done) HIPCHK(E.ctx, hipEventCreateWithFlags(&S.front_done, hipEventDisableTiming));
+  HIPCHK(E.ctx, hipEventRecord(S.front_done, E.ctx->stream));
+  S.front.live = true;
+  S.front.ctx = E.ctx;
+  S.front.b = b;
+  S.front.rows = rows;
+  S.front.stamp = ivf->mutations;
+  return FVDB_OK;
 }
 
 struct StageSpan {
@@ -1181,7 +1251,7 @@
   rc = padded_queries(ivf, E, q_dev, B, &qpad);
   if (rc) return rc;
   HIPCHK(ctx, S.s_qh.ensure((size_t)(B + 1) * ivf->dpad * 2));
-  HIPCHK(ctx, S.s_cnt.ensure((size_t)ivf->nlist * 4));
+  HIPCHK(ctx, S.s_cnt.ensure((size_t)(ivf->nlist + 2) * 4));
   HIPCHK(ctx, S.s_scnt.ensure((size_t)(B + 2) * 4));
   HIPCHK(ctx, S.s_mslots.ensure((size_t)B * 64 * 4));
   launch_prep_queries(ivf, E, qpad, B);
@@ -1828,13 +1898,78 @@
     if (!e) (void)hipEventCreate(&e);
 }
 
-int ivf_search(fvdb_ivf* ivf, const Env& E, const IvfSearch& R) {
+enum BackState : int {
+  BACK_ENQUEUED = FVDB_BACK_ENQUEUED,
+  BACK_WAITING = FVDB_BACK_WAITING,
+  BACK_PAIRED = FVDB_BACK_PAIRED,
+};
+
+int flush_front(fvdb_ivf* ivf, IvfScratch& S) {
+  if (!S.front.live) return FVDB_OK;
+  S.front.live = false;
+  const Env E{S.front.ctx, &S};
+  const Batch& b = S.front.b;
+  MfmaPlan P;
+  int rc = mfma_plan(ivf, E.ctx, ivf_knobs(), b.B, b.k, b.np, &P);
+  if (rc) return rc;
+  rc = mfma_back(ivf, E, P, b, false);
+  if (rc) return rc;
+  ivf->solo_batches += 1;
+  ivf->last_set.store(E.S);
+  ivf->last_ctx.store(E.ctx);
+  return finish_profile(ivf, E, true, true);
+}
+
+bool pair_fits(fvdb_ivf* ivf, const IvfScratch& lead, uint32_t B, uint32_t k, uint32_t np) {
+  const IvfScratch::Front& f = lead.front;
+  if (!f.live || f.stamp != ivf->mutations || f.b.k != k || f.b.np != np) return false;
+  const uint64_t n = (uint64_t)f.b.B + B;
+  if (n > f.rows || !mfma_shape_ok(ivf, (uint32_t)n, k, np)) return false;
+  const uint32_t maxsegs = std::max<uint32_t>(1, cdiv(ivf->max_list_blocks, pick_segb(ivf, (uint32_t)n, np)));
+  return n * np * maxsegs * k < (1ull << 32);
+}
+
+int pair_back(fvdb_ivf* ivf, IvfScratch& SA, IvfScratch& SB) {
+  const IvfScratch::Front fa = SA.front, fb = SB.front;
+  SA.front.live = SB.front.live = false;
+  const Env EA{fa.ctx, &SA}, EB{fb.ctx, &SB, nullptr, &SA, fa.b.B};
+  const IvfKnobs& kn = ivf_knobs();
+  Batch both = fa.b;
+  both.B = fa.b.B + fb.b.B;
+  MfmaPlan P, PA, PB;
+  int rc = mfma_plan(ivf, EA.ctx, kn, both.B, both.k, both.np, &P);
+  if (!rc) rc = mfma_plan(ivf, EA.ctx, kn, fa.b.B, fa.b.k, fa.b.np, &PA);
+  if (!rc) rc = mfma_plan(ivf, EB.ctx, kn, fb.b.B, fb.b.k, fb.b.np, &PB);
+  if (rc) return rc;
+  for (hipEvent_t* e : {&SA.filter_done, &SA.guest_done})
+    if (!*e) HIPCHK(EA.ctx, hipEventCreateWithFlags(e, hipEventDisableTiming));
+  HIPCHK(EA.ctx, hipStreamWaitEvent(EA.ctx->stream, SB.front_done, 0));
+  MfmaScanArgs a = mfma_scan_args(ivf, EA, P, both);
+  rc = mfma_filter(ivf, EA, P, both, &a);
+  if (rc) return rc;
+  HIPCHK(EA.ctx, hipEventRecord(SA.filter_done, EA.ctx->stream));
+  HIPCHK(EB.ctx, hipStreamWaitEvent(EB.ctx->stream, SA.filter_done, 0));
+  rc = mfma_finish(ivf, EA, PA, fa.b);
+  if (!rc) rc = mfma_finish(ivf, EB, PB, fb.b);
+  if (rc) return rc;
+  HIPCHK(EB.ctx, hipEventRecord(SA.guest_done, EB.ctx->stream));
+  SA.guest = true;
+  SA.pending_profile = SB.pending_profile = false;
+  ivf->paired_batches += 2;
+  return FVDB_OK;
+}
+
+int ivf_search_locked(fvdb_ivf* ivf, const Env& E, const IvfSearch& R, IvfScratch* lead = nullptr, int* state = nullptr) {
   fvdb_ctx* ctx = E.ctx;
   IvfScratch& S = *E.S;
+  if (state) *state = BACK_ENQUEUED;
+  int rc = flush_front(ivf, S);
+  if (rc) return rc;
+  if (lead && !lead->front.live) lead = nullptr;
   const uint32_t np = probed_lists(ivf, R.kind, R.nprobe);
   const bool all = R.kind == IvfSearch::ALL, wide = wide_route(R.kind, np);
   if (!ivf->trained) FAIL(ctx, FVDB_E_NOT_TRAINED, "index not trained");
-  int rc = check_k(ctx, R.kind, R.k, np);
+  rc = check_k(ctx, R.kind, R.k, np);
   if (rc) return rc;
   if (wide && ivf->glob_set)
     FAIL(ctx, FVDB_E_UNSUPPORTED, "the wide search (k or nprobe above FVDB_MAX_K) does not serve a shard of a larger index");
@@ -1844,19 +1979,48 @@
   if (!all && (rc = check_rank(ctx, ivf, np))) return rc;
   rc = upload_table(ivf);
   if (rc) return rc;
-  std::lock_guard<std::mutex> enq(S.enq);
+  if (S.guest) {
+    HIPCHK(ctx, hipStreamWaitEvent(ctx->stream, S.guest_done, 0));
+    S.guest = false;
+  }
   ensure_stage_events(ivf, S);
   const uint32_t step = wide ? wide_sub_batch(ivf, R.B, np) : sub_batch(ivf, R.B, R.k, np);
+  const IvfKnobs& kn = ivf_knobs();
+  const int pairing = ivf->pairing.load();
+  const bool may_wait = state && (pairing < 0 ? kn.pair : pairing != 0) && !kn.mfma_threshold_pass && R.kind == IvfSearch::PROBED && !wide && !E.live &&
+                        !R.given_probes && !R.given_thr && step >= R.B;
   for (uint32_t o = 0; o < R.B; o += step) {
     const IvfSearch r = R.slice(o, std::min(step, R.B - o), ivf->d, np);
     const float* qpad = nullptr;
     rc = padded_queries(ivf, E, r.q_dev, r.B, &qpad);
     if (rc) return rc;
-    HIPCHK(ctx, S.s_probes.ensure((size_t)r.B * np * 4));
-    const uint32_t* probes = S.s_probes.as<uint32_t>();
+    const bool fine = R.kind != IvfSearch::COARSE_ONLY;
+    const int role = all ? ROLE_ALL : ROLE_LIST;
+    FineRoute route;
+    if (fine && !wide) route = fine_route(ivf, E, Batch{qpad, nullptr, r.B, r.k, np, nullptr, nullptr, nullptr, nullptr, r.given_thr}, role);
+    const bool wait = may_wait && route.mfma && !route.refine;
+    Env Eb = E;
+    if (lead) {
+      if (wait && pair_fits(ivf, *lead, r.B, r.k, np)) {
+        Eb.Q = lead;
+        Eb.qo = lead->front.b.B;
+        HIPCHK(ctx, hipStreamWaitEvent(ctx->stream, lead->front_done, 0));
+      } else {
+        rc = flush_front(ivf, *lead);
+        if (rc) return rc;
+        lead = nullptr;
+      }
+    }
+    uint32_t* own_probes = nullptr;
+    if (Eb.Q) {
+      own_probes = Eb.Q->s_probes.as<uint32_t>() + (size_t)Eb.qo * np;
+    } else {
+      HIPCHK(ctx, S.s_probes.ensure((size_t)(wait ? pair_rows(r.B) : r.B) * np * 4));
+      own_probes = S.s_probes.as<uint32_t>();
+    }
+    const uint32_t* probes = own_probes;
     if (all) {
-      hipLaunchKernelGGL(probes_all_kernel, dim3(cdiv((uint64_t)r.B * np, 256)), dim3(256), 0, ctx->stream, r.B, np,
-                         S.s_probes.as<uint32_t>());
+      hipLaunchKernelGGL(probes_all_kernel, dim3(cdiv((uint64_t)r.B * np, 256)), dim3(256), 0, ctx->stream, r.B, np, own_probes);
       mark(ivf, E, EV_COARSE_DONE);
     } else if (r.given_probes) {
       probes = r.given_probes;
@@ -1864,19 +2028,32 @@
       mark(ivf, E, EV_COARSE_SCANNED);
       mark(ivf, E, EV_COARSE_DONE);
     } else {
-      rc = run_coarse(ivf, E, qpad, r.B, np, r.probes_out ? r.probes_out : S.s_probes.as<uint32_t>(), nullptr);
+      rc = run_coarse(ivf, E, qpad, r.B, np, r.probes_out ? r.probes_out : own_probes, nullptr);
       if (rc) return rc;
     }
-    if (R.kind == IvfSearch::COARSE_ONLY) continue;
+    if (!fine) continue;
     const Batch b{qpad, probes, r.B, r.k, np, r.ids, r.dist, r.counts, r.keys, r.given_thr};
-    rc = wide ? run_fine_wide(ivf, E, b) : run_fine(ivf, E, b, all ? ROLE_ALL : ROLE_LIST);
+    rc = wide ? run_fine_wide(ivf, E, b) : run_fine(ivf, Eb, b, role, route, wait);
     if (rc) return rc;
+    if (wait) {
+      *state = BACK_WAITING;
+      if (lead) {
+        rc = pair_back(ivf, *lead, S);
+        if (rc) return rc;
+        *state = BACK_PAIRED;
+      }
+      continue;
+    }
     rc = finish_profile(ivf, E, !all, true);
     if (rc) return rc;
   }
   ivf->last_set.store(E.S);
   ivf->last_ctx.store(E.ctx);
   return FVDB_OK;
+}
+int ivf_search(fvdb_ivf* ivf, const Env& E, const IvfSearch& R) {
+  std::lock_guard<std::mutex> enq(E.S->enq);
+  return ivf_search_locked(ivf, E, R);
 }
 
 int slot_env(fvdb_ivf* ivf, fvdb_ctx* on, uint32_t slot, Env* E) {
@@ -1991,6 +2168,55 @@
                              uint64_t* out_keys_dev) {
   return search_on_slot(ivf, on, slot, kNoMask,
                         IvfSearch{IvfSearch::PROBED, q_dev, B, k, nprobe, out_ids_dev, out_dist_dev, out_counts_dev, out_keys_dev});
+}
+
+int fvdb_ivf_search_begin_dev_slot(fvdb_ivf* ivf, fvdb_ctx* on, uint32_t slot, const float* q_dev, uint32_t B, uint32_t k,
+                                   uint32_t nprobe, uint64_t* out_ids_dev, float* out_dist_dev, uint32_t* out_counts_dev,
+                                   int32_t waiting_slot, int* state) {
+  if (!ivf) return FVDB_E_INVALID;
+  if (!state) FAIL(ivf->ctx, FVDB_E_INVALID, "null state");
+  if (waiting_slot >= (int32_t)fvdb_ivf::kSlots) FAIL(ivf->ctx, FVDB_E_INVALID, "slot out of range");
+  return on_slot(ivf, on, slot, kNoMask, [&](const Env& E) -> int {
+    IvfScratch* lead = waiting_slot >= 0 ? &slot_scratch(ivf, (uint32_t)waiting_slot) : nullptr;
+    if (lead == E.S) lead = nullptr;
+    std::unique_lock<std::mutex> own(E.S->enq, std::defer_lock), other;
+    if (lead) {
+      other = std::unique_lock<std::mutex>(lead->enq, std::defer_lock);
+      std::lock(own, other);
+    } else {
+      own.lock();
+    }
+    const IvfSearch R{IvfSearch::PROBED, q_dev, B, k, nprobe, out_ids_dev, out_dist_dev, out_counts_dev};
+    int rc = ivf_search_locked(ivf, E, R, lead, state);
+    if (lead) {
+      const int rcl = flush_front(ivf, *lead);
+      if (!rc) rc = rcl;
+    }
+    return rc;
+  });
+}
+
+int fvdb_ivf_search_flush_slot(fvdb_ivf* ivf, uint32_t slot) {
+  if (!ivf) return FVDB_E_INVALID;
+  if (slot >= fvdb_ivf::kSlots) FAIL(ivf->ctx, FVDB_E_INVALID, "slot out of range");
+  IvfScratch& S = slot_scratch(ivf, slot);
+  std::lock_guard<std::mutex> enq(S.enq);
+  if (!S.front.live) return FVDB_OK;
+  HIPCHK(ivf->ctx, hipSetDevice(ivf->ctx->device));
+  return slot_done(ivf, Env{S.front.ctx, &S}, flush_front(ivf, S));
+}
+
+int fvdb_ivf_set_pairing(fvdb_ivf* ivf, int on) {
+  if (!ivf) return FVDB_E_INVALID;
+  ivf->pairing.store(on < 0 ? -1 : (on ? 1 : 0));
+  return FVDB_OK;
+}
+
+int fvdb_ivf_pair_stats(fvdb_ivf* ivf, uint64_t* paired, uint64_t* alone) {
+  if (!ivf || !paired || !alone) return FVDB_E_INVALID;
+  *paired = ivf->paired_batches.load();
+  *alone = ivf->solo_batches.load();
+  return FVDB_OK;
 }
 
 int fvdb_ivf_search_probes_dev_slot(fvdb_ivf* ivf, fvdb_ctx* on, uint32_t slot, const float* q_dev,
diff --git a/fabstir-vectordb_amd/host/fvdb_host.hpp b/fabstir-vectordb_amd/host/fvdb_host.hpp
--- a/fabstir-vectordb_amd/host/fvdb_host.hpp
+++ b/fabstir-vectordb_amd/host/fvdb_host.hpp
@@ -125,6 +125,9 @@
              uint32_t* counts);
   int search_dev(const float* q_dev, uint32_t B, uint32_t dim, uint32_t k, uint32_t n_probe, uint64_t* ids_dev,
                  float* dist_dev, uint32_t* counts_dev, fvdb_ctx* on = nullptr, uint32_t slot = 0);
+  int search_dev_begin(const float* q_dev, uint32_t B, uint32_t dim, uint32_t k, uint32_t n_probe, uint64_t* ids_dev,
+                       float* dist_dev, uint32_t* counts_dev, fvdb_ctx* on, uint32_t slot, int32_t waiting_slot, int* state);
+  int search_dev_flush(uint32_t slot) { return dev_ ? fvdb_ivf_search_flush_slot(dev_, slot) : FVDB_OK; }
   int search_allowed(const float* q, uint32_t B, uint32_t dim, uint32_t k, uint32_t n_probe, const uint64_t* allowed,
                      uint64_t n_allowed, uint64_t* ids, float* dist, uint32_t* counts);
   int allowed_mask(const uint64_t* allowed, uint64_t n_allowed, MaskRef* out);
@@ -509,6 +512,7 @@
   struct Slot {
     DevBuf ivf;
     uint32_t ivf_rows = 0;
+    uint32_t ivf_slot = 0;
     fvdb_event* ivf_done = nullptr;
     fvdb_ctx* ivf_ctx = nullptr;
     bool active = false, ivf_in_flight = false, hnsw_in_flight = false, recent = false;
@@ -519,6 +523,9 @@
     HNSWIndex::ViewRef view;
   };
   Slot slots_[kSlots];
+  int waiting_slot_ = -1;
+  int flush_waiting_locked();
+  int ivf_chain_complete(Slot& sl);
   struct Lease {
     static constexpr uint32_t kAnyFree = ~0u;
     enum How { kTake, kAdopt };
diff --git a/fabstir-vectordb_amd/host/hybrid_index.cpp b/fabstir-vectordb_amd/host/hybrid_index.cpp
--- a/fabstir-vectordb_amd/host/hybrid_index.cpp
+++ b/fabstir-vectordb_amd/host/hybrid_index.cpp
@@ -538,6 +538,22 @@
 };
 }
 
+int HybridIndex::ivf_chain_complete(Slot& sl) {
+  const uint64_t bytes = IvfBlock::bytes(sl.ivf_rows, sl.hk);
+  if (fvdb_dev_download_async(sl.ivf_ctx, sl.ivf.host, sl.ivf.dev, (size_t)bytes) || fvdb_event_record(sl.ivf_ctx, sl.ivf_done))
+    return FVDB_E_HIP;
+  return FVDB_OK;
+}
+
+int HybridIndex::flush_waiting_locked() {
+  if (waiting_slot_ < 0) return FVDB_OK;
+  Slot& w = slots_[waiting_slot_];
+  waiting_slot_ = -1;
+  const int rc = historical_->search_dev_flush(w.ivf_slot);
+  const int rcc = ivf_chain_complete(w);
+  return rc ? rc : rcc;
+}
+
 int HybridIndex::begin_impl(uint32_t slot, const float* q_dev, uint32_t B, uint32_t dim, const HybridSearchConfig& cfg,
                             int shard_mode) {
   Slot& sl = slots_[slot];
@@ -574,24 +590,39 @@
     if (slot_ctx(ctx_ivf_, slot == 0 || one_stream, &sl.ivf_ctx)) return FVDB_E_HIP;
     fvdb_ctx* on = sl.ivf_ctx == ctx_ivf_ ? nullptr : sl.ivf_ctx;
     if (!sl.ivf_done && fvdb_event_create(sl.ivf_ctx, &sl.ivf_done)) return FVDB_E_HIP;
+    sl.ivf_slot = on ? slot : 0;
     if (shard_mode >= 0) {
       if (dim != historical_->dimension()) return FVDB_E_DIM;
+      {
+        std::lock_guard<std::mutex> lk(slot_mu_);
+        if (int rcw = flush_waiting_locked()) return rcw;
+      }
       const int rcs = fvdb_ivf_search_sharded_begin(sharded_, on, on ? slot : 0, q_dev, B_ivf_in, sl.hk,
                                                     (uint32_t)cfg.ivf_n_probe, shard_mode, d.ids, d.dist, d.counts);
       if (rcs) return rcs;
       sl.ivf_in_flight = true;
-    } else {
-      const int rch = sl.ivf_mask ? historical_->search_dev_masked(sl.ivf_mask, q_dev, B, dim, sl.hk, (uint32_t)cfg.ivf_n_probe,
-                                                                   d.ids, d.dist, d.counts, on, on ? slot : 0)
-                                  : historical_->search_dev(q_dev, B, dim, sl.hk, (uint32_t)cfg.ivf_n_probe, d.ids, d.dist,
-                                                            d.counts, on, on ? slot : 0);
+      return ivf_chain_complete(sl);
+    }
+    std::lock_guard<std::mutex> lk(slot_mu_);
+    if (sl.ivf_mask) {
+      if (int rcw = flush_waiting_locked()) return rcw;
+      const int rch = historical_->search_dev_masked(sl.ivf_mask, q_dev, B, dim, sl.hk, (uint32_t)cfg.ivf_n_probe, d.ids, d.dist,
+                                                     d.counts, on, sl.ivf_slot);
       if (rch) return rch;
       sl.ivf_in_flight = true;
-    }
-    if (sl.ivf_in_flight) {
-      if (fvdb_dev_download_async(sl.ivf_ctx, sl.ivf.host, sl.ivf.dev, (size_t)bytes) || fvdb_event_record(sl.ivf_ctx, sl.ivf_done))
-        return FVDB_E_HIP;
-    }
+      return ivf_chain_complete(sl);
+    }
+    const int waiting = waiting_slot_;
+    int state = FVDB_BACK_ENQUEUED;
+    const int rch = historical_->search_dev_begin(q_dev, B, dim, sl.hk, (uint32_t)cfg.ivf_n_probe, d.ids, d.dist, d.counts, on,
+                                                  sl.ivf_slot, waiting >= 0 ? (int32_t)slots_[waiting].ivf_slot : -1, &state);
+    waiting_slot_ = -1;
+    const int rcw = waiting >= 0 ? ivf_chain_complete(slots_[waiting]) : FVDB_OK;
+    if (rch) return rch;
+    sl.ivf_in_flight = true;
+    if (state == FVDB_BACK_WAITING) waiting_slot_ = (int)slot;
+    else if (int rcc = ivf_chain_complete(sl)) return rcc;
+    return rcw;
   }
   return FVDB_OK;
 }
@@ -602,6 +633,10 @@
   if (!lease.sl) return FVDB_E_INVALID;
   Slot& sl = *lease.sl;
   const uint32_t B = sl.B, k = sl.k;
+  {
+    std::lock_guard<std::mutex> lk(slot_mu_);
+    if (waiting_slot_ == (int)slot) (void)flush_waiting_locked();
+  }
   struct DropMasks {
     Slot& sl;
     ~DropMasks() {
diff --git a/fabstir-vectordb_amd/host/ivf_index.cpp b/fabstir-vectordb_amd/host/ivf_index.cpp
--- a/fabstir-vectordb_amd/host/ivf_index.cpp
+++ b/fabstir-vectordb_amd/host/ivf_index.cpp
@@ -441,6 +441,20 @@
   return fvdb_ivf_search_dev_slot(dev_, on, slot, q_dev, B, k, n_probe, ids_dev, dist_dev, counts_dev, nullptr);
 }
 
+int IVFIndex::search_dev_begin(const float* q_dev, uint32_t B, uint32_t dim, uint32_t k, uint32_t n_probe, uint64_t* ids_dev,
+                               float* dist_dev, uint32_t* counts_dev, fvdb_ctx* on, uint32_t slot, int32_t waiting_slot,
+                               int* state) {
+  *state = FVDB_BACK_ENQUEUED;
+  int rc = !trained_ ? FVDB_E_NOT_TRAINED : (dim != dim_ ? FVDB_E_DIM : FVDB_OK);
+  if (rc || k > FVDB_MAX_K) {
+    const int rcw = waiting_slot >= 0 ? search_dev_flush((uint32_t)waiting_slot) : FVDB_OK;
+    if (rc) return rc;
+    rc = fvdb_ivf_search_wide_dev_slot(dev_, on, slot, nullptr, q_dev, B, k, n_probe, ids_dev, dist_dev, counts_dev, nullptr);
+    return rc ? rc : rcw;
+  }
+  return fvdb_ivf_search_begin_dev_slot(dev_, on, slot, q_dev, B, k, n_probe, ids_dev, dist_dev, counts_dev, waiting_slot, state);
+}
+
 int IVFIndex::allowed_mask(const uint64_t* allowed, uint64_t n_allowed, MaskRef* out) {
   if (!trained_ || !dev_) return FVDB_E_NOT_TRAINED;
   if (n_allowed && !allowed) return FVDB_E_INVALID;
diff --git a/include/fvdb.h b/include/fvdb.h
--- a/include/fvdb.h
+++ b/include/fvdb.h
@@ -123,6 +123,15 @@
 int fvdb_ivf_search_dev_slot(fvdb_ivf* ivf, fvdb_ctx* on, uint32_t slot, const float* q_dev, uint32_t B, uint32_t k,
                              uint32_t nprobe, uint64_t* out_ids_dev, float* out_dist_dev, uint32_t* out_counts_dev,
                              uint64_t* out_keys_dev);
+#define FVDB_BACK_ENQUEUED 0
+#define FVDB_BACK_WAITING 1
+#define FVDB_BACK_PAIRED 2
+int fvdb_ivf_search_begin_dev_slot(fvdb_ivf* ivf, fvdb_ctx* on, uint32_t slot, const float* q_dev, uint32_t B, uint32_t k,
+                                   uint32_t nprobe, uint64_t* out_ids_dev, float* out_dist_dev, uint32_t* out_counts_dev,
+                                   int32_t waiting_slot, int* state);
+int fvdb_ivf_search_flush_slot(fvdb_ivf* ivf, uint32_t slot);
+int fvdb_ivf_set_pairing(fvdb_ivf* ivf, int on);
+int fvdb_ivf_pair_stats(fvdb_ivf* ivf, uint64_t* paired, uint64_t* alone);
 int fvdb_ivf_coarse_dev_slot(fvdb_ivf* ivf, fvdb_ctx* on, uint32_t slot, const float* q_dev, uint32_t B, uint32_t nprobe,
                              uint32_t* out_probes_dev);
 int fvdb_ivf_search_probes_dev_slot(fvdb_ivf* ivf, fvdb_ctx* on, uint32_t slot, const float* q_dev,
```

Result: slower. 1.690 million (-5.5%).
